# Geo3DSmart/PDANet

Hardware: AMD Instinct MI355X
Metric: scenes/sec (16384-pt ONCE, PDA-SSD forward+backward) (higher is better)
Workload: dtype f32; 1 GPU; once16k_b2_detector_fwd_bwd_adam; scenes_per_gpu=2, global_batch=2, parallelism=dp1, world_size_seen=1, cpu_affinity=GPU-local NUMA node of 0000:d9:00.0: 128 CPUs, full=False, graph_tail=False, graph_head=True

## Files before the change

include/pda_pointnet2.h:

```cpp
#ifndef PDA_POINTNET2_H
#define PDA_POINTNET2_H

#include <stdint.h>

#ifdef __cplusplus
extern "C" {
#endif

#define PDA_OK 0
#define PDA_ERR_INVALID_ARGUMENT 1
#define PDA_ERR_LAUNCH 2
#define PDA_ERR_UNSUPPORTED 3

typedef void *pda_stream_t;

#define PDA_POINTNET2_ABI_VERSION 20
int pda_abi_version(void);
const char *pda_last_error(void);
int pda_fp_contract_mode(void);
int pda_opt_n_threads(int work_size);
int pda_fps_coop_timeouts(unsigned long long *total, int reset);
int pda_debug_fps_spin_limit(int polls);
long long pda_debug_fps_exchange_nonzero(void);

// ... 25 lines not shown
int pda_group_points(const float *points, const int32_t *idx, float *out, int b, int c, int n,
                     int npoints, int nsample, pda_stream_t stream);
int pda_group_points_grad(const float *grad_out, const int32_t *idx, float *grad_points, int b,
                          int c, int n, int npoints, int nsample, pda_stream_t stream);

int pda_group_rows(const float *rows, const int32_t *idx, float *out, int b, int n, int c,
                   int64_t num_idx, pda_stream_t stream);
int pda_group_rows_grad(const float *grad_out, const int32_t *idx, float *grad_rows, int b, int n,
                        int c, int64_t num_idx, pda_stream_t stream);

int pda_three_nn(const float *unknown, const float *known, float *dist2, int32_t *idx, int b,
                 int n, int m, pda_stream_t stream);
int pda_three_interpolate(const float *points, const int32_t *idx, const float *weight,
                          float *out, int b, int c, int m, int n, pda_stream_t stream);
int pda_three_interpolate_grad(const float *grad_out, const int32_t *idx, const float *weight,
                               float *grad_points, int b, int c, int n, int m,
                               pda_stream_t stream);

int pda_chamfer_forward(const float *xyz1, const float *xyz2, float *dist1, float *dist2,
                        int32_t *idx1, int32_t *idx2, int b, int n, int m, pda_stream_t stream);
int pda_chamfer_backward(const float *xyz1, const float *xyz2, float *gradxyz1, float *gradxyz2,
                         const float *graddist1, const float *graddist2, const int32_t *idx1,
                         const int32_t *idx2, int b, int n, int m, pda_stream_t stream);

int pda_group_attention_fwd(const float *qkv, float *out, float *lse, int64_t num_groups, int seq,
                            int heads, int head_dim, pda_stream_t stream);
int pda_group_attention_bwd(const float *qkv, const float *grad_out, const float *lse,
                            float *grad_qkv, int64_t num_groups, int seq, int heads, int head_dim,
                            pda_stream_t stream);
int pda_group_attention_fwd_bf16(const uint16_t *qkv, uint16_t *out, float *lse, int64_t num_groups, int seq,
                                 int heads, int head_dim, pda_stream_t stream);
int pda_group_attention_bwd_bf16(const uint16_t *qkv, const uint16_t *grad_out, const float *lse,
                                 uint16_t *grad_qkv, int64_t num_groups, int seq, int heads, int head_dim,
                                 pda_stream_t stream);

int pda_sa_mlp_maxpool(const float *xyz, const float *new_xyz, const float *features,
                       const int32_t *idx, float *out, int b, int n, int m, int c, int nsample,
                       const int32_t *dims, const float *const *wf, const float *const *scale,
                       const float *const *shift, pda_stream_t stream);
int pda_linear_cols_packed_size(int n_out, int k);
int pda_linear_cols_pack(const float *w, float *wf, int n_out, int k, int transposed_source, int gather_order,
                         pda_stream_t stream);
int pda_linear_cols(const float *x, const float *wf, float *y, int64_t tokens, int k, int n_out, pda_stream_t stream);
int pda_sa_gather_linear(const float *xyz, const float *new_xyz, const float *feats_pm, const int32_t *idx,
                         const float *wf, float *y, int b, int n, int m, int c, int nsample, int n_out,
                         pda_stream_t stream);
int64_t pda_linear_split_packed_bytes(int n_out, int k);
int pda_linear_split_pack(const float *w, void *wf, int n_out, int k, int transposed_source, pda_stream_t stream);
int pda_linear_split_pack_both(const float *w, void *wf, void *wft, int n_out, int k, pda_stream_t stream);
int pda_linear_split(const float *x, const void *wf, const float *bias, float *y, int64_t tokens, int k, int n_out,
                     int relu, pda_stream_t stream);
int pda_gemm_split(const float *x, const void *wf, const float *bias, float *y, int64_t tokens, int k, int n_out,
                   int relu, int accumulate, pda_stream_t stream);
int pda_sa_mlp_packed_size(int rows, int cols, int first_layer);
int pda_sa_mlp_pack_weights(const float *w, float *wf, int rows, int cols, int first_layer,
                            pda_stream_t stream);

#ifdef __cplusplus
}
#endif
#endif
```

include/pda_train.h:

```cpp
#ifndef PDA_TRAIN_H
#define PDA_TRAIN_H
#include "pda_pointnet2.h"

#ifdef __cplusplus
extern "C" {
#endif

int pda_grad_norm(const float *g, int64_t n, float *norm_out, float *scratch1024, pda_stream_t stream);
int pda_adam_onecycle_step(float *p, const float *g, float *m, float *v, int64_t n, float lr,
                           float beta1, float beta2, float eps, float wd, int step,
                           const float *total_norm, float max_norm, pda_stream_t stream);

int64_t pda_bn_relu_scratch_bytes(int c);
int pda_bn_relu_fwd(const float *x, const float *gamma, const float *beta, float *running_mean,
                    float *running_var, float *y, float *mean_invstd, void *scratch, int64_t rows, int c,
                    float eps, float momentum, pda_stream_t stream);
int pda_bn_relu_bwd(const float *x, const float *grad_y, const float *gamma, const float *beta,
                    const float *mean_invstd, float *grad_x, float *grad_gamma, float *grad_beta,
                    void *scratch, int64_t rows, int c, pda_stream_t stream);
int pda_bn_relu_fwd_mixed(const void *x, int x_is_bf16, const float *gamma, const float *beta, float *running_mean,
                          float *running_var, void *y, int y_is_bf16, float *mean_invstd, void *scratch,
                          int64_t rows, int c, float eps, float momentum, pda_stream_t stream);
int pda_bn_relu_bwd_mixed(const void *x, int x_is_bf16, const void *grad_y, int grad_y_is_bf16, const float *gamma,
                          const float *beta, const float *mean_invstd, void *grad_x, float *grad_gamma,
                          float *grad_beta, void *scratch, int64_t rows, int c, pda_stream_t stream);
int pda_bn_relu_max_pool_fwd(const void *x, int x_is_bf16, const float *gamma, const float *beta, float *running_mean,
                             float *running_var, float *out, uint8_t *arg, float *mean_invstd, void *scratch,
                             int64_t groups, int ns, int c, float eps, float momentum, pda_stream_t stream);
int pda_bn_relu_max_pool_bwd(const void *x, int x_is_bf16, const float *grad_out, const uint8_t *arg,
                             const float *gamma, const float *beta, const float *mean_invstd, void *grad_x,
                             float *grad_gamma, float *grad_beta, void *scratch, int64_t groups, int ns, int c,
                             pda_stream_t stream);

int64_t pda_layer_norm_scratch_bytes(int d);
int pda_layer_norm_fwd(const float *x, const float *residual, const float *gamma, const float *beta,
                       float *sum_out, float *y, float *mean_rstd, int64_t rows, int d, float eps,
                       pda_stream_t stream);
int pda_layer_norm_bwd(const float *x, const float *grad_y, const float *grad_y2, const float *gamma,
                       const float *mean_rstd, float *grad_x, float *grad_gamma, float *grad_beta,
                       void *scratch, int64_t rows, int d, pda_stream_t stream);
int pda_layer_norm_fwd_mixed(const void *x, int x_is_bf16, const float *residual, const float *gamma,
                             const float *beta, float *sum_out, float *y, uint16_t *y_bf16, float *mean_rstd,
                             int64_t rows, int d, float eps, pda_stream_t stream);
int pda_layer_norm_bwd_mixed(const float *x, const float *grad_y, const void *grad_y2, int grad_y2_is_bf16,
                             const float *gamma, const float *mean_rstd, float *grad_x, uint16_t *grad_x_bf16,
                             float *grad_gamma, float *grad_beta, void *scratch, int64_t rows, int d,
                             pda_stream_t stream);

int64_t pda_linear_wgrad_scratch_bytes(int64_t tokens, int in_features, int out_features);
int pda_linear_wgrad_form(int64_t tokens, int in_features, int out_features);
int pda_linear_wgrad(const float *x, const float *grad_out, float *grad_weight, float *grad_bias,
                     void *scratch, int64_t tokens, int in_features, int out_features, pda_stream_t stream);
int pda_linear_wgrad_bn(const float *x, const float *grad_out, float *grad_weight, float *grad_bias, void *scratch,
                        int64_t tokens, int in_features, int out_features, const float *x_mean_invstd,
                        const float *x_gamma, const float *x_beta, pda_stream_t stream);

int64_t pda_gemm_split_bn_tiles(int64_t tokens);
int pda_gemm_split_bn(const float *x, const void *wf, float *y, int64_t tokens, int k, int n_out,
                      const float *in_mean_invstd, const float *in_gamma, const float *in_beta, int stats_mode,
                      double *partial, pda_stream_t stream);
int pda_gemm_split_maxpool(const float *x, const void *wf, const float *bias, float *out, int64_t tokens, int k, int n_out,
                           int ns, int relu, pda_stream_t stream);
int pda_gemm_split_gather(const float *point_rows, const float *xyz, const float *new_xyz, const int32_t *idx,
                          const float *w1, int ldw1, const float *bias1, const void *wf, const float *bias2, float *y,
                          int b, int n, int m, int ns, int k, int n_out, int relu, pda_stream_t stream);
int pda_bn_stats_fwd(const float *x, float *running_mean, float *running_var, float *mean_invstd, void *scratch,
                     int64_t rows, int c, float eps, float momentum, pda_stream_t stream);
int pda_bn_finalize_fwd(const double *partial, int nblocks, int c, int64_t count, float eps, float momentum,
                        float *mean_invstd, float *running_mean, float *running_var, pda_stream_t stream);
int pda_bn_relu_max_pool_apply(const float *x, const float *gamma, const float *beta, const float *mean_invstd,
                               float *out, uint8_t *arg, int64_t groups, int ns, int c, pda_stream_t stream);

int64_t pda_colsum_scratch_bytes(int cols);
int pda_colsum_bf16(const uint16_t *g, float *out, void *scratch, int64_t rows, int cols, pda_stream_t stream);

int pda_assemble_tokens(const float *rppe, const float *dscale, const float *feats, const int32_t *idx,
                        const float *glob, float *out, int b, int n, int m, int nsample, int c,
                        pda_stream_t stream);
int pda_assemble_tokens_grad(const float *grad_out, const float *dscale, const float *feats, const int32_t *idx,
                             float *grad_rppe, float *grad_dscale, float *grad_feats, float *grad_glob,
                             int b, int n, int m, int nsample, int c, pda_stream_t stream);

int pda_add_max_pool(const float *a, const float *b, float *out, uint8_t *arg, int64_t groups, int seq, int d,
                     pda_stream_t stream);
int pda_max_pool_scatter(const float *grad_out, const uint8_t *arg, float *grad_x, int64_t groups, int seq,
                         int d, pda_stream_t stream);
int pda_add_max_pool_bf16(const float *a, const uint16_t *b, float *out, uint8_t *arg, int64_t groups, int seq,
                          int d, pda_stream_t stream);
int pda_max_pool_scatter_bf16(const float *grad_out, const uint8_t *arg, float *grad_x, uint16_t *grad_x_bf16,
                              int64_t groups, int seq, int d, pda_stream_t stream);

int pda_bn_relu_fwd_weighted(const float *x, const float *gamma, const float *beta, float *running_mean,
                             float *running_var, float *y, float *mean_invstd, void *scratch, int64_t rows, int c,
                             float eps, float momentum, const float *row_weight, int64_t count, pda_stream_t stream);
int pda_bn_relu_bwd_weighted(const float *x, const float *grad_y, const float *gamma, const float *beta,
                             const float *mean_invstd, float *grad_x, float *grad_gamma, float *grad_beta,
                             void *scratch, int64_t rows, int c, const float *row_weight, int64_t count,
                             pda_stream_t stream);

int pda_ragged_plan(const int32_t *idx, int32_t *cnt, int32_t *off, int32_t *rowmap, float *row_weight, int64_t groups,
                    int nsample, pda_stream_t stream);
int pda_assemble_tokens_ragged(const float *rppe, const float *dscale, const float *feats, const int32_t *idx,
                               const float *glob, const int32_t *rowmap, const int32_t *off, float *out,
                               int64_t max_tokens, int b, int n, int m, int nsample, int c, int rppe_compact,
                               pda_stream_t stream);
int pda_assemble_tokens_ragged_grad(const float *grad_out, const float *dscale, const float *feats,
                                    const int32_t *idx, const int32_t *cnt, const int32_t *off, const int32_t *rowmap,
                                    float *grad_rppe, float *grad_dscale, float *grad_feats, float *grad_glob,
// ... 305 lines not shown
```

pdanet_amd/_lib.py:

```python
import ctypes
import os

_HERE = os.path.dirname(os.path.abspath(__file__))
LIB_PATH = os.environ.get("PDA_LIB_PATH") or os.path.join(_HERE, "libpda_pointnet2.so")
ABI_VERSION = 20


class DensityNetScale(ctypes.Structure):
    _fields_ = [("x", ctypes.c_void_p), ("grad_y", ctypes.c_void_p), ("params", ctypes.c_void_p), ("y", ctypes.c_void_p),
                ("stats", ctypes.c_void_p), ("scratch", ctypes.c_void_p), ("running", ctypes.c_void_p * 6),
                ("grad_params", ctypes.c_void_p), ("n", ctypes.c_int64), ("rowmap", ctypes.c_void_p),
                ("row_weight", ctypes.c_void_p), ("n_unique", ctypes.c_void_p), ("nsample", ctypes.c_int),
                ("eps", ctypes.c_float), ("momentum", ctypes.c_float)]


class OnceFrames(ctypes.Structure):
    _fields_ = [("gt_boxes", ctypes.c_void_p), ("gt_name", ctypes.c_void_p), ("gt_offsets", ctypes.c_void_p),
                ("pred_boxes", ctypes.c_void_p), ("pred_score", ctypes.c_void_p), ("pred_name", ctypes.c_void_p),
                ("pred_start", ctypes.c_void_p), ("pred_count", ctypes.c_void_p), ("iou_start", ctypes.c_void_p),
                ("n_gt_total", ctypes.c_int64), ("pred_cap", ctypes.c_int64), ("iou_cap", ctypes.c_int64),
                ("n_frames", ctypes.c_int), ("max_gt", ctypes.c_int), ("max_pred", ctypes.c_int)]


class KittiFrames(ctypes.Structure):
    _fields_ = [(n, ctypes.c_void_p) for n in ("gt_bbox", "gt_loc", "gt_dims", "gt_ry", "gt_alpha", "gt_trunc", "gt_occ",
                                               "gt_name", "gt_offsets", "dt_bbox", "dt_box", "dt_alpha", "dt_score",
                                               "dt_name", "dt_start", "dt_count", "ov_start", "frame_mode")] + \
               [("n_gt_total", ctypes.c_int64), ("det_cap", ctypes.c_int64), ("ov_cap", ctypes.c_int64),
                ("n_frames", ctypes.c_int), ("max_gt", ctypes.c_int), ("max_det", ctypes.c_int)]


PARAM_EPOCH = [0]
WEIGHT_EPOCH = [0]

_vp = ctypes.c_void_p
_i = ctypes.c_int
_f = ctypes.c_float

SIGNATURES = {
    "pda_furthest_point_sampling": [_vp, _vp, _vp, _i, _i, _i, _vp],
    "pda_furthest_point_sampling_with_dist": [_vp, _vp, _vp, _i, _i, _i, _vp],
    "pda_gather_points": [_vp, _vp, _vp, _i, _i, _i, _i, _vp],
    "pda_gather_points_grad": [_vp, _vp, _vp, _i, _i, _i, _i, _vp],
    "pda_ball_query": [_vp, _vp, _vp, _i, _i, _i, _f, _i, _vp],
    "pda_ball_query_dilated": [_vp, _vp, _vp, _i, _i, _i, _f, _f, _i, _vp],
    "pda_ellipsoid_query": [_vp, _vp, _vp, _i, _i, _i, _f, _f, _f, _i, _vp],
    "pda_ball_query_cells_scratch_bytes": [_i, _i],
    "pda_ball_query_cells": [_vp, _vp, ctypes.POINTER(_vp), _i, _i, _i, _i, ctypes.POINTER(_f), ctypes.POINTER(ctypes.c_int32),
                             _vp, ctypes.c_int64, _vp],
    "pda_ball_query_multi": [_vp, _vp, ctypes.POINTER(_vp), _i, _i, _i, _i,
                             ctypes.POINTER(_f), ctypes.POINTER(ctypes.c_int32), _vp],
    "pda_group_points": [_vp, _vp, _vp, _i, _i, _i, _i, _i, _vp],
    "pda_group_points_grad": [_vp, _vp, _vp, _i, _i, _i, _i, _i, _vp],
    "pda_group_rows": [_vp, _vp, _vp, _i, _i, _i, ctypes.c_int64, _vp],
    "pda_group_rows_grad": [_vp, _vp, _vp, _i, _i, _i, ctypes.c_int64, _vp],
    "pda_three_nn": [_vp, _vp, _vp, _vp, _i, _i, _i, _vp],
    "pda_three_interpolate": [_vp, _vp, _vp, _vp, _i, _i, _i, _i, _vp],
    "pda_three_interpolate_grad": [_vp, _vp, _vp, _vp, _i, _i, _i, _i, _vp],
    "pda_chamfer_forward": [_vp, _vp, _vp, _vp, _vp, _vp, _i, _i, _i, _vp],
    "pda_chamfer_backward": [_vp, _vp, _vp, _vp, _vp, _vp, _vp, _vp, _i, _i, _i, _vp],
    "pda_group_attention_fwd": [_vp, _vp, _vp, ctypes.c_int64, _i, _i, _i, _vp],
    "pda_group_attention_bwd": [_vp, _vp, _vp, _vp, ctypes.c_int64, _i, _i, _i, _vp],
    "pda_group_attention_fwd_bf16": [_vp, _vp, _vp, ctypes.c_int64, _i, _i, _i, _vp],
    "pda_group_attention_bwd_bf16": [_vp, _vp, _vp, _vp, ctypes.c_int64, _i, _i, _i, _vp],
    "pda_sa_mlp_maxpool": [_vp, _vp, _vp, _vp, _vp, _i, _i, _i, _i, _i, ctypes.POINTER(ctypes.c_int32),
                           ctypes.POINTER(_vp), ctypes.POINTER(_vp), ctypes.POINTER(_vp), _vp],
    "pda_linear_cols_packed_size": [_i, _i],
    "pda_linear_cols_pack": [_vp, _vp, _i, _i, _i, _i, _vp],
    "pda_linear_cols": [_vp, _vp, _vp, ctypes.c_int64, _i, _i, _vp],
    "pda_sa_gather_linear": [_vp, _vp, _vp, _vp, _vp, _vp, _i, _i, _i, _i, _i, _i, _vp],
    "pda_linear_split_packed_bytes": [_i, _i],
    "pda_linear_split_pack": [_vp, _vp, _i, _i, _i, _vp],
    "pda_linear_split_pack_both": [_vp, _vp, _vp, _i, _i, _vp],
    "pda_linear_split": [_vp, _vp, _vp, _vp, ctypes.c_int64, _i, _i, _i, _vp],
    "pda_gemm_split": [_vp, _vp, _vp, _vp, ctypes.c_int64, _i, _i, _i, _i, _vp],
    "pda_sa_mlp_packed_size": [_i, _i, _i],
    "pda_sa_mlp_pack_weights": [_vp, _vp, _i, _i, _i, _vp],
    "pda_grad_norm": [_vp, ctypes.c_int64, _vp, _vp, _vp],
    "pda_bn_relu_scratch_bytes": [_i],
    "pda_bn_relu_fwd": [_vp, _vp, _vp, _vp, _vp, _vp, _vp, _vp, ctypes.c_int64, _i, _f, _f, _vp],
    "pda_bn_relu_bwd": [_vp, _vp, _vp, _vp, _vp, _vp, _vp, _vp, _vp, ctypes.c_int64, _i, _vp],    "pda_bn_relu_fwd_mixed": [_vp, _i, _vp, _vp, _vp, _vp, _vp, _i, _vp, _vp, ctypes.c_int64, _i, _f, _f, _vp],
    "pda_bn_relu_bwd_mixed": [_vp, _i, _vp, _i, _vp, _vp, _vp, _vp, _vp, _vp, _vp, ctypes.c_int64, _i, _vp],
    "pda_bn_relu_max_pool_fwd": [_vp, _i, _vp, _vp, _vp, _vp, _vp, _vp, _vp, _vp, ctypes.c_int64, _i, _i, _f, _f, _vp],
    "pda_bn_relu_max_pool_bwd": [_vp, _i, _vp, _vp, _vp, _vp, _vp, _vp, _vp, _vp, _vp, ctypes.c_int64, _i, _i, _vp],

    "pda_layer_norm_scratch_bytes": [_i],
    "pda_layer_norm_fwd": [_vp, _vp, _vp, _vp, _vp, _vp, _vp, ctypes.c_int64, _i, _f, _vp],
    "pda_layer_norm_bwd": [_vp, _vp, _vp, _vp, _vp, _vp, _vp, _vp, _vp, ctypes.c_int64, _i, _vp],
    "pda_layer_norm_fwd_mixed": [_vp, _i, _vp, _vp, _vp, _vp, _vp, _vp, _vp, ctypes.c_int64, _i, _f, _vp],
    "pda_layer_norm_bwd_mixed": [_vp, _vp, _vp, _i, _vp, _vp, _vp, _vp, _vp, _vp, _vp, ctypes.c_int64, _i, _vp],
    "pda_linear_wgrad_scratch_bytes": [ctypes.c_int64, _i, _i],
    "pda_linear_wgrad_form": [ctypes.c_int64, _i, _i],
    "pda_linear_wgrad": [_vp, _vp, _vp, _vp, _vp, ctypes.c_int64, _i, _i, _vp],
    "pda_linear_wgrad_bn": [_vp, _vp, _vp, _vp, _vp, ctypes.c_int64, _i, _i, _vp, _vp, _vp, _vp],
    "pda_gemm_split_bn_tiles": [ctypes.c_int64],
    "pda_gemm_split_bn": [_vp, _vp, _vp, ctypes.c_int64, _i, _i, _vp, _vp, _vp, _i, _vp, _vp],
    "pda_gemm_split_maxpool": [_vp, _vp, _vp, _vp, ctypes.c_int64, _i, _i, _i, _i, _vp],
    "pda_gemm_split_gather": [_vp, _vp, _vp, _vp, _vp, _i, _vp, _vp, _vp, _vp, _i, _i, _i, _i, _i, _i, _i, _vp],
    "pda_bn_stats_fwd": [_vp, _vp, _vp, _vp, _vp, ctypes.c_int64, _i, _f, _f, _vp],
    "pda_bn_finalize_fwd": [_vp, _i, _i, ctypes.c_int64, _f, _f, _vp, _vp, _vp, _vp],
    "pda_bn_relu_max_pool_apply": [_vp, _vp, _vp, _vp, _vp, _vp, ctypes.c_int64, _i, _i, _vp],
    "pda_colsum_scratch_bytes": [_i],
    "pda_colsum_bf16": [_vp, _vp, _vp, ctypes.c_int64, _i, _vp],
    "pda_assemble_tokens": [_vp, _vp, _vp, _vp, _vp, _vp, _i, _i, _i, _i, _i, _vp],
    "pda_assemble_tokens_grad": [_vp, _vp, _vp, _vp, _vp, _vp, _vp, _vp, _i, _i, _i, _i, _i, _vp],
    "pda_add_max_pool": [_vp, _vp, _vp, _vp, ctypes.c_int64, _i, _i, _vp],
    "pda_max_pool_scatter": [_vp, _vp, _vp, ctypes.c_int64, _i, _i, _vp],
    "pda_add_max_pool_bf16": [_vp, _vp, _vp, _vp, ctypes.c_int64, _i, _i, _vp],
    "pda_max_pool_scatter_bf16": [_vp, _vp, _vp, _vp, ctypes.c_int64, _i, _i, _vp],
    "pda_ragged_plan": [_vp, _vp, _vp, _vp, _vp, ctypes.c_int64, _i, _vp],
    "pda_assemble_tokens_ragged": [_vp, _vp, _vp, _vp, _vp, _vp, _vp, _vp, ctypes.c_int64, _i, _i, _i, _i, _i, _i, _vp],
    "pda_assemble_tokens_ragged_grad": [_vp, _vp, _vp, _vp, _vp, _vp, _vp, _vp, _vp, _vp, _vp, ctypes.c_int64, _i, _i, _i, _i, _i, _i, _vp],
    "pda_bn_relu_fwd_weighted": [_vp, _vp, _vp, _vp, _vp, _vp, _vp, _vp, ctypes.c_int64, _i, _f, _f, _vp, ctypes.c_int64, _vp],
    "pda_bn_relu_bwd_weighted": [_vp, _vp, _vp, _vp, _vp, _vp, _vp, _vp, _vp, ctypes.c_int64, _i, _vp, ctypes.c_int64, _vp],
    "pda_add_max_pool_ragged": [_vp, _vp, _vp, _vp, _vp, _vp, ctypes.c_int64, _i, _vp],
    "pda_max_pool_scatter_ragged": [_vp, _vp, _vp, _vp, _vp, ctypes.c_int64, ctypes.c_int64, _i, _i, _vp],
    "pda_group_attention_ragged_fwd": [_vp, _vp, _vp, _vp, _vp, ctypes.c_int64, ctypes.c_int64, _i, _i, _i, _vp],
    "pda_group_attention_ragged_bwd": [_vp, _vp, _vp, _vp, _vp, _vp, ctypes.c_int64, ctypes.c_int64, _i, _i, _i, _vp],
    "pda_densitynet_param_count": [],
    "pda_densitynet_eval_param_count": [],
    "pda_densitynet_scratch_bytes": [],
    "pda_densitynet_fwd": [_vp, _vp, _vp, _vp, _vp, _vp, _vp, _vp, _vp, _vp, _vp, ctypes.c_int64, _f, _f, _vp],
    "pda_densitynet_bwd": [_vp, _vp, _vp, _vp, _vp, _vp, ctypes.c_int64, _f, _vp],
    "pda_densitynet_eval": [_vp, _vp, _vp, ctypes.c_int64, _vp],
    "pda_densitynet_fwd_multi": [_vp, _i, _vp],
    "pda_densitynet_bwd_multi": [_vp, _i, _vp],
    "pda_densitynet_fwd_unique": [_vp, _vp, _vp, _vp, _vp, _vp, _vp, _vp, _vp, _vp, _vp, ctypes.c_int64, _vp, _vp, _vp, _i, _f, _f, _vp],
    "pda_densitynet_bwd_unique": [_vp, _vp, _vp, _vp, _vp, _vp, ctypes.c_int64, _vp, _vp, _vp, _i, _f, _vp],
    "pda_pda_geometry": [_vp, _vp, _vp, _vp, _vp, _i, _i, _i, _i, _f, _vp],
    "pda_points_in_boxes": [_vp, _vp, _vp, _i, _i, _i, _vp],
    "pda_roiaware_pool3d_fwd": [_vp, _vp, _vp, _vp, _vp, _vp, _i, _i, _i, _i, _i, _i, _i, _i, _vp],
    "pda_roiaware_pool3d_bwd": [_vp, _vp, _vp, _vp, _i, _i, _i, _i, _i, _i, _i, _i, _vp],
    "pda_roipoint_pool3d_fwd": [_vp, _vp, _vp, _vp, _vp, _i, _i, _i, _i, _i, _vp],
    "pda_points_in_boxes_mask": [_vp, _vp, _vp, _i, _i, _vp],
    "pda_assign_point_targets": [_vp, _vp, _vp, _vp, _vp, _vp, _i, _i, _i, _i, _i, _vp],
    "pda_sa_gaussian_mask": [_vp, _i, _i, _vp, _vp, _vp, ctypes.c_int64, _vp],
    "pda_head_assign_targets": [_vp, _i, _i, _vp, ctypes.POINTER(ctypes.c_float), _vp, _vp, _vp, _vp, _vp, _i, _i, _i, _i, _i, _i, _vp],
    "pda_head_cls_loss": [_vp, _i, _i, _i, _vp, _vp, ctypes.c_int64, _f, _vp, _vp, _vp],
    "pda_head_centerness": [_vp, _vp, _vp, _vp, ctypes.c_int64, _vp],
    "pda_head_box_loss": [_vp, _vp, _vp, _vp, _f, _i, _f, _f, ctypes.c_int64, _vp, _vp, _vp],
    "pda_head_vote_loss": [_i, _vp, _vp, _vp, _vp, _i, _i, _i, _f, ctypes.c_int64, _vp, _vp, _vp],
    "pda_head_corner_loss": [_vp, _vp, _vp, _i, _vp, _vp, _vp, _i, _f, ctypes.c_int64, _vp, _vp, _vp, _vp],
    "pda_boxes_overlap_bev": [_vp, _vp, _vp, _i, _i, _vp],
    "pda_boxes_iou_bev": [_vp, _vp, _vp, _i, _i, _vp],
    "pda_nms_mask_words": [_i],
    "pda_nms_bev": [_vp, _vp, _vp, _vp, _vp, _i, _i, _f, _i, _vp],
    "pda_sa_small_train_workspace_bytes": [],
# ... 161 lines not shown
```

pdanet_amd/csrc/gemm_split.hip:

```cpp
#include "pda_common.h"
#include "split_bf16.h"

#include <stdlib.h>

namespace pda {

constexpr int GS_MAX_N = 2048;
constexpr int GS_KSTEP = 12 * 64;

__device__ __forceinline__ void split_pack_one(const float* __restrict__ w, uint32_t* __restrict__ wf, int64_t o, int rows, int cols,
                                               int KS, int trans) {
    const int pr = (int)(o & 3), lane = (int)((o >> 2) & 63);
    int64_t rest = o >> 8;
    const int rb = (int)(rest & 3); rest >>= 2;
    const int s = (int)(rest % KS), c = (int)(rest / KS);
    const int row = c * 128 + rb * 32 + (lane & 31);
    const int k = 16 * s + 8 * (lane >> 5) + 2 * pr;
    float v[2];
    for (int e = 0; e < 2; ++e)
        v[e] = (row < rows && k + e < cols) ? (trans ? w[(size_t)(k + e) * rows + row] : w[(size_t)row * cols + k + e]) : 0.f;
    uint32_t h, m, l;
    split2(v[0], v[1], h, m, l);
    const size_t base = ((((size_t)c * KS + s) * 4 + rb) * 3) * 256 + (size_t)lane * 4 + pr;
    wf[base] = h; wf[base + 256] = m; wf[base + 512] = l;
}

__global__ void split_pack_kernel(const float* __restrict__ w, uint32_t* __restrict__ wf, int rows, int cols, int KS,
                                  int chunks, int trans) {
    const int64_t total = (int64_t)chunks * KS * 4 * 64 * 4;
    for (int64_t o = blockIdx.x * (int64_t)blockDim.x + threadIdx.x; o < total; o += (int64_t)gridDim.x * blockDim.x)
        split_pack_one(w, wf, o, rows, cols, KS, trans);
}

__global__ void split_pack_both_kernel(const float* __restrict__ w, uint32_t* __restrict__ wf, uint32_t* __restrict__ wft, int n_out,
                                       int k, int KS, int chunks, int KSt, int chunks_t) {
    const int64_t total = (int64_t)chunks * KS * 4 * 64 * 4, total_t = (int64_t)chunks_t * KSt * 4 * 64 * 4;
    for (int64_t o = blockIdx.x * (int64_t)blockDim.x + threadIdx.x; o < total + total_t; o += (int64_t)gridDim.x * blockDim.x) {
        if (o < total) split_pack_one(w, wf, o, n_out, k, KS, 0);
        else split_pack_one(w, wft, o - total, k, n_out, KSt, 1);
    }
}

struct LinSplitParams {
    const float* x;
    const uint4* wf;
    const float* bias;
    float* y;
    int64_t tokens;
    int k, n_out, chunks, relu;
    int cpb;
    unsigned long long* dbg;
};
#ifdef GS_PROFILE
#define GS_MARK(i) do { if (tid == 0) p.dbg[(size_t)blockIdx.x * 16 + (i)] = __builtin_readcyclecounter(); } while (0)
#else
#define GS_MARK(i) do {} while (0)
#endif

template <int KS>
__global__ __launch_bounds__(256) __attribute__((amdgpu_waves_per_eu(1, 1)))
void lin_split_kernel(const LinSplitParams p) {
    constexpr int G = KS % 4 == 0 ? 4 : 2;
    constexpr int TILE = G * GS_KSTEP;
    constexpr int NG = KS / G;
    constexpr int NLD = TILE / 256;
    __shared__ uint4 ring[3 * TILE];
    __shared__ float bias_s[GS_MAX_N];
    const int tid = threadIdx.x, lane = tid & 63, w = __builtin_amdgcn_readfirstlane(tid >> 6);
    const int h = lane >> 5, j = lane & 31;
    const int64_t tok0 = ((int64_t)blockIdx.x * 4 + w) * 32;
    const int64_t tk = tok0 + j < p.tokens ? tok0 + j : p.tokens - 1;
    const uint4* src = p.wf + tid;
    const int ntiles = p.chunks * NG;
    const int c0 = (int)blockIdx.y * p.cpb, c1 = min(p.chunks, c0 + p.cpb);
    const uint32_t ring_base = (uint32_t)(uintptr_t)(__attribute__((address_space(3))) void*)ring + w * 1024;
    auto issue = [&](int t, int slot) {
        const uint4* g = src + (size_t)(t < ntiles ? t : ntiles - 1) * TILE;
        const uint32_t l = ring_base + slot * (TILE * 16);
#pragma unroll
        for (int i = 0; i < NLD; ++i) glds16(g + 256 * i, l + 4096 * i);
    };
    static_assert(NLD <= G * 4, "one DMA instruction per MFMA group at most");
    GS_MARK(0);
    float x[KS * 8];
    {
        const float* row = p.x + tk * p.k + 8 * h;
#pragma unroll
        for (int s = 0; s < KS; ++s) {
            const float4 a = *reinterpret_cast<const float4*>(row + 16 * s), b = *reinterpret_cast<const float4*>(row + 16 * s + 4);
            x[8 * s] = a.x; x[8 * s + 1] = a.y; x[8 * s + 2] = a.z; x[8 * s + 3] = a.w;
            x[8 * s + 4] = b.x; x[8 * s + 5] = b.y; x[8 * s + 6] = b.z; x[8 * s + 7] = b.w;
        }
    }
    for (int i = tid; i < p.n_out; i += 256) bias_s[i] = p.bias ? p.bias[i] : 0.f;
    asm volatile("s_waitcnt vmcnt(0)" ::: "memory");
    GS_MARK(1);
    issue(c0 * NG, 0);
    issue(c0 * NG + 1, 1);
    asm volatile("s_waitcnt vmcnt(%0)" ::"n"(NLD) : "memory");
    __builtin_amdgcn_s_barrier();
    GS_MARK(2);
    const uint32_t lane_off = (uint32_t)(4 * h * p.n_out + j);
    const int64_t left = p.tokens - tok0 - 4 * h;
    const bool whole = tok0 + 32 <= p.tokens;
    auto store_one = [&](const gs_f32x16 (&res)[4], int chunk, int n) {
        const int r = n >> 4, i = n & 15, t = (i & 3) + 8 * (i >> 2);
        float v = res[r][i] + bias_s[chunk * 128 + r * 32 + j];
        if (p.relu) v = fmaxf(v, 0.f);
        float* row = p.y + (tok0 + t) * p.n_out + chunk * 128 + r * 32;
        if (whole) row[lane_off] = v;
        else if (t < left) row[lane_off] = v;
    };
    int ti = c0 * NG, slot = 0;
    gs_f32x16 done[4];
    for (int c = c0; c < c1; ++c) {
        gs_f32x16 acc[4];
#pragma unroll
        for (int r = 0; r < 4; ++r)
#pragma unroll
            for (int i = 0; i < 16; ++i) acc[r][i] = 0.f;
#pragma unroll
        for (int g = 0; g < NG; ++g, ++ti, slot = slot == 2 ? 0 : slot + 1) {
            if (c == 1 && g == 0) GS_MARK(4);
            const uint4* dsrc = src + (size_t)(ti + 2 < ntiles ? ti + 2 : ntiles - 1) * TILE;
            const uint32_t ddst = ring_base + (slot == 0 ? 2 : slot - 1) * (TILE * 16);
            if (c == 1 && g == 0) GS_MARK(5);
            const uint4* buf = ring + slot * TILE + lane;
            uint4 fa[2][3];
#pragma unroll
            for (int pl = 0; pl < 3; ++pl) fa[0][pl] = buf[pl * 64];
#pragma unroll
            for (int sl = 0; sl < G; ++sl) {
                const int s = g * G + sl;
                if constexpr (KS > 16) {
#pragma unroll
                    for (int q = 0; q < 8; ++q) asm volatile("" : "+v"(x[8 * s + q]));
                }
                uint32_t bh[4], bm[4], bl[4];
#pragma unroll
                for (int q = 0; q < 4; ++q) split2(x[8 * s + 2 * q], x[8 * s + 2 * q + 1], bh[q], bm[q], bl[q]);
                const gs_bf16x8 Xh = __builtin_bit_cast(gs_bf16x8, make_uint4(bh[0], bh[1], bh[2], bh[3]));
                const gs_bf16x8 Xm = __builtin_bit_cast(gs_bf16x8, make_uint4(bm[0], bm[1], bm[2], bm[3]));
                const gs_bf16x8 Xl = __builtin_bit_cast(gs_bf16x8, make_uint4(bl[0], bl[1], bl[2], bl[3]));
#pragma unroll
                for (int r = 0; r < 4; ++r) {
                    const int q = sl * 4 + r;
                    if (q + 1 < G * 4) {
#pragma unroll
                        for (int pl = 0; pl < 3; ++pl) fa[(q + 1) & 1][pl] = buf[((q + 1) * 3 + pl) * 64];
                    }
                    __builtin_amdgcn_sched_barrier(0);
                    const gs_bf16x8 Wh = __builtin_bit_cast(gs_bf16x8, fa[q & 1][0]);
                    const gs_bf16x8 Wm = __builtin_bit_cast(gs_bf16x8, fa[q & 1][1]);
                    const gs_bf16x8 Wl = __builtin_bit_cast(gs_bf16x8, fa[q & 1][2]);
                    acc[r] = __builtin_amdgcn_mfma_f32_32x32x16_bf16(Xl, Wh, acc[r], 0, 0, 0);
                    acc[r] = __builtin_amdgcn_mfma_f32_32x32x16_bf16(Xh, Wl, acc[r], 0, 0, 0);
                    acc[r] = __builtin_amdgcn_mfma_f32_32x32x16_bf16(Xm, Wm, acc[r], 0, 0, 0);
                    acc[r] = __builtin_amdgcn_mfma_f32_32x32x16_bf16(Xm, Wh, acc[r], 0, 0, 0);
                    acc[r] = __builtin_amdgcn_mfma_f32_32x32x16_bf16(Xh, Wm, acc[r], 0, 0, 0);
                    acc[r] = __builtin_amdgcn_mfma_f32_32x32x16_bf16(Xh, Wh, acc[r], 0, 0, 0);
                    if (q < NLD) glds16(dsrc + 256 * q, ddst + 4096 * q);
                    if (c > c0) {
                        constexpr int GROUPS = KS * 4;
                        const int gq = g * G * 4 + q;
#pragma unroll
                        for (int n = gq * 64 / GROUPS; n < (gq + 1) * 64 / GROUPS; ++n) store_one(done, c - 1, n);
                    }
                    __builtin_amdgcn_sched_barrier(0);
                }
            }
            if (c == 1 && g == 0) GS_MARK(6);
            asm volatile("s_waitcnt vmcnt(%0)" ::"n"(NLD) : "memory");
            if (c == 1 && g == 0) GS_MARK(7);
            __builtin_amdgcn_s_barrier();
            if (c == 1 && g == 0) GS_MARK(8);
            if (c == 0 && g == NG - 1) GS_MARK(3);
        }
#pragma unroll
        for (int r = 0; r < 4; ++r) done[r] = acc[r];
    }
    GS_MARK(9);
#pragma unroll
    for (int n = 0; n < 64; ++n) store_one(done, c1 - 1, n);
    GS_MARK(10);
}

struct GemmSplitParams {
    const float* x;
    const uint4* wf;
    const float* bias;
    float* y;
    int64_t tokens;
    int k, n_out, chunks, ksteps, relu, accum;
    const float* in_mi;
    const float* in_g;
    const float* in_b;
    double* partial;
    int pool_ns;
    const int32_t* g_idx;
    const float* g_xyz;
    const float* g_ctr;
    const float* g_w;
    const float* g_bias;
    int gn, g_ns, g_m, g_ldw;
};

constexpr int GT_XCHUNKS = 128 * 4;
constexpr int GT_SLOT = GT_XCHUNKS + GS_KSTEP;
constexpr int GW_TILE_U4 = (8 + 8) * 192;

__global__ __launch_bounds__(256, 2)
void gemm_split_kernel(const GemmSplitParams p) {
    __shared__ uint4 ring[3 * GT_SLOT];
    const int tid = threadIdx.x, lane = tid & 63, w = __builtin_amdgcn_readfirstlane(tid >> 6);
    const int h = lane >> 5, r = lane & 31;
    const int wt = w & 1, wo = w >> 1;
    const int nc = (int)(blockIdx.x % (unsigned)p.chunks);
    const int64_t tok0 = (int64_t)(blockIdx.x / (unsigned)p.chunks) * 128;
    const uint32_t ring_base = (uint32_t)(uintptr_t)(__attribute__((address_space(3))) void*)ring;
    const float* xsrc[2];
#pragma unroll
    for (int e = 0; e < 2; ++e) {
        const int pch = 64 * (2 * w + e) + lane, row = pch >> 2, cl = pch & 3, c = cl ^ ((row >> 2) & 3);
        const int64_t tok = tok0 + row < p.tokens ? tok0 + row : p.tokens - 1;
        xsrc[e] = p.x + tok * p.k + 4 * c;
    }
    const uint4* wsrc = p.wf + (size_t)nc * p.ksteps * GS_KSTEP + 64 * 3 * w + lane;
    auto issue = [&](int s, int slot) {
        const int ss = s < p.ksteps ? s : p.ksteps - 1;
        const uint32_t base = ring_base + slot * (GT_SLOT * 16);
#pragma unroll
        for (int e = 0; e < 2; ++e) glds16(reinterpret_cast<const uint4*>(xsrc[e] + 16 * ss), base + (2 * w + e) * 1024);
#pragma unroll
        for (int e = 0; e < 3; ++e) glds16(wsrc + (size_t)ss * GS_KSTEP + 64 * e, base + GT_XCHUNKS * 16 + (3 * w + e) * 1024);
    };
    gs_f32x16 acc[2][2];
#pragma unroll
    for (int a = 0; a < 2; ++a)
#pragma unroll
        for (int b = 0; b < 2; ++b)
#pragma unroll
            for (int i = 0; i < 16; ++i) acc[a][b][i] = 0.f;
    int xoff[2][2];
#pragma unroll
    for (int tt = 0; tt < 2; ++tt) {
        const int row = wt * 64 + tt * 32 + r;
// ... 12 lines not shown
        const uint4* buf = ring + slot * GT_SLOT;
        uint4 wfr[2][3];
#pragma unroll
        for (int ot = 0; ot < 2; ++ot)
#pragma unroll
            for (int pl = 0; pl < 3; ++pl) wfr[ot][pl] = buf[woff + (ot * 3 + pl) * 64];
#pragma unroll
        for (int tt = 0; tt < 2; ++tt) {
            const uint4 a = buf[xoff[tt][0]], b = buf[xoff[tt][1]];
            uint32_t bh[4], bm[4], bl[4];
#ifdef GS_NOSPLIT
            bh[0] = a.x; bh[1] = a.y; bh[2] = a.z; bh[3] = a.w; bm[0] = b.x; bm[1] = b.y; bm[2] = b.z; bm[3] = b.w;
            bl[0] = a.x ^ b.x; bl[1] = a.y ^ b.y; bl[2] = a.z ^ b.z; bl[3] = a.w ^ b.w;
#else
            split2(__uint_as_float(a.x), __uint_as_float(a.y), bh[0], bm[0], bl[0]);
            split2(__uint_as_float(a.z), __uint_as_float(a.w), bh[1], bm[1], bl[1]);
            split2(__uint_as_float(b.x), __uint_as_float(b.y), bh[2], bm[2], bl[2]);
            split2(__uint_as_float(b.z), __uint_as_float(b.w), bh[3], bm[3], bl[3]);
#endif
            const gs_bf16x8 Xh = __builtin_bit_cast(gs_bf16x8, make_uint4(bh[0], bh[1], bh[2], bh[3]));
            const gs_bf16x8 Xm = __builtin_bit_cast(gs_bf16x8, make_uint4(bm[0], bm[1], bm[2], bm[3]));
            const gs_bf16x8 Xl = __builtin_bit_cast(gs_bf16x8, make_uint4(bl[0], bl[1], bl[2], bl[3]));
#pragma unroll
            for (int ot = 0; ot < 2; ++ot) {
                const gs_bf16x8 Wh = __builtin_bit_cast(gs_bf16x8, wfr[ot][0]);
                const gs_bf16x8 Wm = __builtin_bit_cast(gs_bf16x8, wfr[ot][1]);
                const gs_bf16x8 Wl = __builtin_bit_cast(gs_bf16x8, wfr[ot][2]);
                gs_f32x16 c = acc[tt][ot];
                c = __builtin_amdgcn_mfma_f32_32x32x16_bf16(Xl, Wh, c, 0, 0, 0);
                c = __builtin_amdgcn_mfma_f32_32x32x16_bf16(Xh, Wl, c, 0, 0, 0);
                c = __builtin_amdgcn_mfma_f32_32x32x16_bf16(Xm, Wm, c, 0, 0, 0);
                c = __builtin_amdgcn_mfma_f32_32x32x16_bf16(Xm, Wh, c, 0, 0, 0);
                c = __builtin_amdgcn_mfma_f32_32x32x16_bf16(Xh, Wm, c, 0, 0, 0);
                c = __builtin_amdgcn_mfma_f32_32x32x16_bf16(Xh, Wh, c, 0, 0, 0);
                acc[tt][ot] = c;
            }
        }
    }
    asm volatile("s_waitcnt vmcnt(0)" ::: "memory");
#pragma unroll
    for (int ot = 0; ot < 2; ++ot) {
        const int col = nc * 128 + (wo * 2 + ot) * 32 + r;
        if (col >= p.n_out) continue;
        const float bias = p.bias ? p.bias[col] : 0.f;
#pragma unroll
        for (int tt = 0; tt < 2; ++tt) {
            const int64_t trow = tok0 + wt * 64 + tt * 32 + 4 * h;
#pragma unroll
            for (int i = 0; i < 16; ++i) {
                const int64_t tok = trow + (i & 3) + 8 * (i >> 2);
                if (tok < p.tokens) {
                    float* dst = p.y + tok * p.n_out + col;
                    float v = acc[tt][ot][i] + bias;
                    if (p.accum) v += *dst;
                    if (p.relu) v = fmaxf(v, 0.f);
#ifdef GS_NOSTORE
                    if (v == 12345.678f)
#endif
                    *dst = v;
                }
            }
        }
    }
}

typedef uint32_t gp_u32x4 __attribute__((ext_vector_type(4)));

template <int PRO, int EPI>
__global__ __launch_bounds__(512, 1)
void gemm_split_wide_kernel(const GemmSplitParams p) {
    constexpr int TW = 4;
    constexpr int XF = 2 * TW;
    constexpr int NP = 24 / (2 * TW);
    constexpr int TILE_U4 = GW_TILE_U4;
    extern __shared__ uint4 gp_planes[];
    const int tid = threadIdx.x, lane = tid & 63, w = __builtin_amdgcn_readfirstlane(tid >> 6);
    const int h = lane >> 5, r = lane & 31;
    const int wt = w % TW, wo = w / TW;
    const int wide_chunks = (p.chunks + 1) >> 1;
    const int ncb = (int)(blockIdx.x % (unsigned)wide_chunks);
    const int64_t tok0 = (int64_t)(blockIdx.x / (unsigned)wide_chunks) * (64 * TW);
    const int64_t ptok = tok0 + 32 * w + r < p.tokens ? tok0 + 32 * w + r : p.tokens - 1;
    const float* xsrc = p.x + ptok * p.k + 8 * h;
    float gdx = 0.f, gdy = 0.f, gdz = 0.f;
    if constexpr (PRO == 2) {
        const int64_t grp = ptok / p.g_ns;
        const int64_t prow = (grp / p.g_m) * p.gn + p.g_idx[ptok];
        xsrc = p.x + prow * p.k + 8 * h;
        const float* pt = p.g_xyz + prow * 3;
        const float* ct = p.g_ctr + grp * 3;
        gdx = pt[0] - ct[0]; gdy = pt[1] - ct[1]; gdz = pt[2] - ct[2];
    }
    const uint4* wsrc[NP];
#pragma unroll
    for (int e = 0; e < NP; ++e) {
        const int piece = NP * w + e, half = piece / 12, j = piece - 12 * half;
        int chunk = 2 * ncb + half;
        if (chunk >= p.chunks) chunk = p.chunks - 1;
        wsrc[e] = p.wf + (size_t)chunk * p.ksteps * GS_KSTEP + 64 * j + lane;
    }
    auto wld = [&](int e, int ss) { return *reinterpret_cast<const gp_u32x4*>(wsrc[e] + (size_t)ss * GS_KSTEP); };
    auto wst = [&](uint4* dst, const gp_u32x4& v) { *reinterpret_cast<gp_u32x4*>(dst) = v; };
    auto load = [&](int st, float4 (&x)[2], gp_u32x4 (&wv)[NP]) {
        const int ss = st < p.ksteps ? st : p.ksteps - 1;
        x[0] = *reinterpret_cast<const float4*>(xsrc + 16 * ss);
        x[1] = *reinterpret_cast<const float4*>(xsrc + 16 * ss + 4);
#pragma unroll
// ... 135 lines not shown
    if constexpr (EPI == 2) {
        const int ns = p.pool_ns;
#pragma unroll
        for (int ot = 0; ot < 4; ++ot) {
            const int col = (2 * ncb + wo) * 128 + ot * 32 + r;
            const float bias = (p.bias && col < p.n_out) ? p.bias[col] : 0.f;
            float g16[4];
#pragma unroll
            for (int tt = 0; tt < 2; ++tt)
#pragma unroll
                for (int half = 0; half < 2; ++half) {
                    float m = -__builtin_inff();
#pragma unroll
                    for (int i = 8 * half; i < 8 * half + 8; ++i) {
                        float v = acc[tt][ot][i] + bias;
                        if (p.relu) v = fmaxf(v, 0.f);
                        m = fmaxf(m, v);
                    }
                    g16[2 * tt + half] = fmaxf(m, __shfl_xor(m, 32));
                }
            if (h == 0 && col < p.n_out) {
                const int64_t t0 = tok0 + wt * 64;
                if (ns == 16) {
#pragma unroll
                    for (int q = 0; q < 4; ++q)
                        if (t0 + 16 * q < p.tokens) p.y[((t0 + 16 * q) >> 4) * p.n_out + col] = g16[q];
                } else if (ns == 32) {
#pragma unroll
                    for (int q = 0; q < 2; ++q)
                        if (t0 + 32 * q < p.tokens) p.y[((t0 + 32 * q) >> 5) * p.n_out + col] = fmaxf(g16[2 * q], g16[2 * q + 1]);
                } else if (t0 < p.tokens) {
                    p.y[(t0 >> 6) * p.n_out + col] = fmaxf(fmaxf(g16[0], g16[1]), fmaxf(g16[2], g16[3]));
                }
            }
        }
        return;
    }
    double cs1[4], cs2[4];
#pragma unroll
    for (int ot = 0; ot < 4; ++ot) {
        cs1[ot] = 0; cs2[ot] = 0;
        const int col = (2 * ncb + wo) * 128 + ot * 32 + r;
        if (col >= p.n_out) continue;
        const float bias = p.bias ? p.bias[col] : 0.f;
#pragma unroll
        for (int tt = 0; tt < 2; ++tt) {
            const int64_t trow = tok0 + wt * 64 + tt * 32 + 4 * h;
#pragma unroll
            for (int i = 0; i < 16; ++i) {
                const int64_t tok = trow + (i & 3) + 8 * (i >> 2);
                if (tok < p.tokens) {
                    float* dst = p.y + tok * p.n_out + col;
                    float v = acc[tt][ot][i] + bias;
                    if (p.accum) v += *dst;
                    if (p.relu) v = fmaxf(v, 0.f);
#ifdef GS_NOSTORE
                    if (v == 12345.678f)
#endif
                    *dst = v;
                    if constexpr (EPI == 1) { cs1[ot] += v; cs2[ot] += (double)v * v; }
                }
            }
        }
    }
    if constexpr (EPI == 1) {
        double* red = reinterpret_cast<double*>(gp_planes);
        __syncthreads();
#pragma unroll
        for (int ot = 0; ot < 4; ++ot) {
            const double a = cs1[ot] + __shfl_xor(cs1[ot], 32), b = cs2[ot] + __shfl_xor(cs2[ot], 32);
            if (h == 0) {
                const int cl = wo * 128 + ot * 32 + r;
                red[(wt * 256 + cl) * 2] = a; red[(wt * 256 + cl) * 2 + 1] = b;
            }
        }
        __syncthreads();
        if (tid < 256) {
            const int col = 2 * ncb * 128 + tid;
            if (col < p.n_out) {
                double a = 0, b = 0;
#pragma unroll
                for (int q = 0; q < TW; ++q) { a += red[(q * 256 + tid) * 2]; b += red[(q * 256 + tid) * 2 + 1]; }
                double* pp = p.partial + (size_t)(blockIdx.x / (unsigned)wide_chunks) * 2 * p.n_out;
                pp[col] = a; pp[p.n_out + col] = b;
            }
        }
    }
}

}

PDA_API int64_t pda_linear_split_packed_bytes(int n_out, int k) {
    if (n_out <= 0 || k <= 0) return 0;
    return (int64_t)pda::divup(n_out, 128) * pda::divup(k, 32) * 2 * 12 * 64 * 16;
}

PDA_API int pda_linear_split_pack(const float* w, void* wf, int n_out, int k, int transposed_source, pda_stream_t stream) {
    PDA_REQUIRE(w && wf && n_out > 0 && k > 0, "pda_linear_split_pack: bad argument");
    const int chunks = pda::divup(n_out, 128), KS = pda::divup(k, 32) * 2;
    const int64_t total = (int64_t)chunks * KS * 4 * 64 * 4;
    const int blocks = (int)(pda::divup64(total, 256) < 2048 ? pda::divup64(total, 256) : 2048);
    hipLaunchKernelGGL(pda::split_pack_kernel, dim3(blocks), dim3(256), 0, (hipStream_t)stream, w, (uint32_t*)wf, n_out, k, KS,
                       chunks, transposed_source);
    return pda::check_launch("pda_linear_split_pack");
}

PDA_API int pda_linear_split_pack_both(const float* w, void* wf, void* wft, int n_out, int k, pda_stream_t stream) {
    PDA_REQUIRE(w && wf && wft && n_out > 0 && k > 0, "pda_linear_split_pack_both: bad argument");
    const int chunks = pda::divup(n_out, 128), KS = pda::divup(k, 32) * 2;
    const int chunks_t = pda::divup(k, 128), KSt = pda::divup(n_out, 32) * 2;
    const int64_t total = ((int64_t)chunks * KS + (int64_t)chunks_t * KSt) * 4 * 64 * 4;
    const int blocks = (int)(pda::divup64(total, 256) < 2048 ? pda::divup64(total, 256) : 2048);
    hipLaunchKernelGGL(pda::split_pack_both_kernel, dim3(blocks), dim3(256), 0, (hipStream_t)stream, w, (uint32_t*)wf, (uint32_t*)wft,
                       n_out, k, KS, chunks, KSt, chunks_t);
    return pda::check_launch("pda_linear_split_pack_both");
}

PDA_API int pda_linear_split(const float* x, const void* wf, const float* bias, float* y, int64_t tokens, int k, int n_out,
                             int relu, pda_stream_t stream) {
    PDA_REQUIRE(tokens >= 0 && k > 0 && n_out > 0, "pda_linear_split: bad size");
    if (tokens == 0) return PDA_OK;
    PDA_REQUIRE(x && wf && y && (((uintptr_t)x | (uintptr_t)wf | (uintptr_t)y | (uintptr_t)bias) & 15) == 0,
                "pda_linear_split: null or misaligned pointer");
    if (k % 32 != 0 || k > 512 || n_out % 128 != 0 || n_out > pda::GS_MAX_N) {
        pda::set_error("pda_linear_split: no kernel built for K=%d, N=%d (K a multiple of 32 <= 512, N a multiple of 128 <= 2048)", k, n_out);
        return PDA_ERR_UNSUPPORTED;
    }
    pda::LinSplitParams p{};
    p.x = x; p.wf = (const uint4*)wf; p.bias = bias; p.y = y; p.tokens = tokens; p.k = k; p.n_out = n_out; p.chunks = n_out / 128;
    p.relu = relu;
#ifdef GS_PROFILE
    p.dbg = (unsigned long long*)bias; p.bias = nullptr;
#endif
    const int64_t tiles = pda::divup64(tokens, 128);
    const int want = tiles >= 192 ? 1 : (int)pda::divup64(256, tiles);
    p.cpb = pda::divup(p.chunks, want < p.chunks ? want : p.chunks);
    const dim3 grid((unsigned)tiles, (unsigned)pda::divup(p.chunks, p.cpb)), block(256);
    const hipStream_t s = (hipStream_t)stream;
    switch (k / 16) {
#define PDA_GS_CASE(KS) case KS: hipLaunchKernelGGL((pda::lin_split_kernel<KS>), grid, block, 0, s, p); break
        PDA_GS_CASE(2); PDA_GS_CASE(4); PDA_GS_CASE(6); PDA_GS_CASE(8); PDA_GS_CASE(12); PDA_GS_CASE(16); PDA_GS_CASE(24); PDA_GS_CASE(32);
#undef PDA_GS_CASE
        default:
            pda::set_error("pda_linear_split: no kernel built for K=%d", k);
            return PDA_ERR_UNSUPPORTED;
    }
    return pda::check_launch("pda_linear_split");
}

PDA_API int pda_gemm_split(const float* x, const void* wf, const float* bias, float* y, int64_t tokens, int k, int n_out,
                           int relu, int accumulate, pda_stream_t stream) {
    PDA_REQUIRE(tokens >= 0 && k > 0 && n_out > 0, "pda_gemm_split: bad size");
    if (tokens == 0) return PDA_OK;
    PDA_REQUIRE(x && wf && y && (((uintptr_t)x | (uintptr_t)wf) & 15) == 0, "pda_gemm_split: null or misaligned pointer");
    if (k % 16 != 0) {
        pda::set_error("pda_gemm_split: K=%d must be a multiple of 16", k);
        return PDA_ERR_UNSUPPORTED;
    }
    pda::GemmSplitParams p{};
    p.x = x; p.wf = (const uint4*)wf; p.bias = bias; p.y = y; p.tokens = tokens; p.k = k; p.n_out = n_out;
    p.chunks = pda::divup(n_out, 128); p.ksteps = pda::divup(k, 32) * 2; p.relu = relu; p.accum = accumulate;
    const int64_t blocks = pda::divup64(tokens, 128) * p.chunks;
    PDA_REQUIRE(blocks < (1ll << 31), "pda_gemm_split: too many tiles");
    const int packed_steps = p.ksteps;
    p.ksteps = k / 16;
    if (packed_steps != p.ksteps) {
        pda::set_error("pda_gemm_split: K=%d must be a multiple of 32 (packed planes come in pairs of K steps)", k);
        return PDA_ERR_UNSUPPORTED;
    }
    static const int force = getenv("PDA_GEMM_SPLIT_TILE") ? atoi(getenv("PDA_GEMM_SPLIT_TILE")) : 0;
    const int64_t wide_blocks = pda::divup64(tokens, 256) * ((p.chunks + 1) / 2);
    if (force == 256 || (force != 128 && wide_blocks >= 200 && (p.chunks % 2 == 0 || p.chunks >= 5))) {
        static pda::PerDevice<bool> lds_ok;
        const bool ok = lds_ok.get([] { return hipFuncSetAttribute((const void*)pda::gemm_split_wide_kernel<0, 0>, hipFuncAttributeMaxDynamicSharedMemorySize,
                                                                   2 * pda::GW_TILE_U4 * 16) == hipSuccess; });
        if (ok) {
            hipLaunchKernelGGL((pda::gemm_split_wide_kernel<0, 0>), dim3((unsigned)wide_blocks), dim3(512), 2 * pda::GW_TILE_U4 * 16,
                               (hipStream_t)stream, p);
            return pda::check_launch("pda_gemm_split");
        }
    }
    hipLaunchKernelGGL(pda::gemm_split_kernel, dim3((unsigned)blocks), dim3(256), 0, (hipStream_t)stream, p);
    return pda::check_launch("pda_gemm_split");
}

PDA_API int64_t pda_gemm_split_bn_tiles(int64_t tokens) { return tokens > 0 ? pda::divup64(tokens, 256) : 0; }

PDA_API int pda_gemm_split_bn(const float* x, const void* wf, float* y, int64_t tokens, int k, int n_out, const float* in_mean_invstd,
                              const float* in_gamma, const float* in_beta, int stats_mode, double* partial, pda_stream_t stream) {
    PDA_REQUIRE(tokens >= 1 && k > 0 && n_out > 0, "pda_gemm_split_bn: bad size");
    PDA_REQUIRE(x && wf && y && (((uintptr_t)x | (uintptr_t)wf) & 15) == 0, "pda_gemm_split_bn: null or misaligned pointer");
    const bool pro = in_mean_invstd != nullptr;
    PDA_REQUIRE(pro == (in_gamma != nullptr) && pro == (in_beta != nullptr), "pda_gemm_split_bn: the input BatchNorm needs mean_invstd, gamma and beta");
    PDA_REQUIRE(stats_mode >= 0 && stats_mode <= 1 && (stats_mode == 0 || partial), "pda_gemm_split_bn: stats_mode=%d (0 or 1; 1 needs `partial`)", stats_mode);
    if (k % 32 != 0 || k > 1024) {
        pda::set_error("pda_gemm_split_bn: no kernel built for K=%d (a multiple of 32, <= 1024)", k);
        return PDA_ERR_UNSUPPORTED;
    }
    pda::GemmSplitParams p{};
    p.x = x; p.wf = (const uint4*)wf; p.y = y; p.tokens = tokens; p.k = k; p.n_out = n_out;
    p.chunks = pda::divup(n_out, 128); p.ksteps = k / 16;
    p.in_mi = in_mean_invstd; p.in_g = in_gamma; p.in_b = in_beta; p.partial = partial;
    const int64_t wide_blocks = pda::divup64(tokens, 256) * ((p.chunks + 1) / 2);
    PDA_REQUIRE(wide_blocks < (1ll << 31), "pda_gemm_split_bn: too many tiles");
    const int lds = 2 * pda::GW_TILE_U4 * 16 + (pro ? k * 16 : 0);
    const void* fn;
    if (pro && stats_mode == 1) fn = (const void*)pda::gemm_split_wide_kernel<1, 1>;
    else if (pro && stats_mode == 0) fn = (const void*)pda::gemm_split_wide_kernel<1, 0>;
    else if (stats_mode == 1) fn = (const void*)pda::gemm_split_wide_kernel<0, 1>;
    else fn = (const void*)pda::gemm_split_wide_kernel<0, 0>;
    static pda::PerDevice<bool> lds_ok[4];
    const bool ok = lds_ok[(pro ? 2 : 0) + stats_mode].get([fn] {
        return hipFuncSetAttribute(fn, hipFuncAttributeMaxDynamicSharedMemorySize, 2 * pda::GW_TILE_U4 * 16 + 1024 * 16) == hipSuccess; });
    PDA_REQUIRE(ok, "pda_gemm_split_bn: dynamic LDS refused");
    void* args[] = {(void*)&p};
    PDA_REQUIRE(hipLaunchKernel(fn, dim3((unsigned)wide_blocks), dim3(512), args, lds, (hipStream_t)stream) == hipSuccess,
                "pda_gemm_split_bn: launch failed");
    return pda::check_launch("pda_gemm_split_bn");
}

PDA_API int pda_gemm_split_maxpool(const float* x, const void* wf, const float* bias, float* out, int64_t tokens, int k, int n_out, int ns,
                                   int relu, pda_stream_t stream) {
    PDA_REQUIRE(tokens >= 0 && k > 0 && n_out > 0, "pda_gemm_split_maxpool: bad size");
// ... 46 lines not shown
```

pdanet_amd/csrc/wgrad.hip:

```cpp
#include "pda_common.h"
#include "split_bf16.h"

#include <stdlib.h>

namespace pda {

typedef float f32x16 __attribute__((ext_vector_type(16)));

constexpr int WG_KC = 32;
constexpr int WG_TILE = 128;

__device__ __forceinline__ void lds_dma16(const float* gsrc, float* lds_dst_wave_uniform) {
    uint32_t keep;
    const uint32_t dst = __builtin_amdgcn_readfirstlane((uint32_t)(uintptr_t)lds_dst_wave_uniform);
    asm volatile("s_mov_b32 %0, m0\n\ts_mov_b32 m0, %2\n\ts_nop 0\n\tglobal_load_lds_dwordx4 %1, off\n\ts_mov_b32 m0, %0"
                 : "=&s"(keep) : "v"(gsrc), "s"(dst) : "memory");
}

__global__ __launch_bounds__(256) void wgrad_kernel(const float* __restrict__ X, const float* __restrict__ G,
                                                    float* __restrict__ part_w, float* __restrict__ part_b, int64_t T, int M,
                                                    int N, int tiles_m, int tiles_n, int S, int64_t KS, int nblocks) {
    __shared__ __attribute__((aligned(16))) float ldsG[2][WG_KC][WG_TILE];
    __shared__ __attribute__((aligned(16))) float ldsX[2][WG_KC][WG_TILE];
    const int per_xcd = (nblocks + 7) / 8;
    const int logical = (int)(blockIdx.x & 7) * per_xcd + (int)(blockIdx.x >> 3);
    if (logical >= nblocks) return;
    const int tiles = tiles_m * tiles_n;
    const int tile = logical % tiles, s = logical / tiles;
    const int n0 = (tile / tiles_m) * WG_TILE, m0 = (tile % tiles_m) * WG_TILE;
    const int64_t t_begin = (int64_t)s * KS, t_end = (t_begin + KS < T) ? t_begin + KS : T;

    const int tid = threadIdx.x, lane = lane_id(), w = wave_id();
    const int c = lane & 31, h = lane >> 5;
    const int wn = w >> 1, wm = w & 1;
    const int lrow = tid >> 5, lcol = (tid & 31) * 4;
    const bool g_ok = n0 + lcol < N, x_ok = m0 + lcol < M;

    f32x16 acc[2][2];
#pragma unroll
    for (int i = 0; i < 2; ++i)
#pragma unroll
        for (int j = 0; j < 2; ++j)
#pragma unroll
            for (int r = 0; r < 16; ++r) acc[i][j][r] = 0.f;
    float bsum[2] = {0.f, 0.f};

    float4 rg[4], rx[4];
    const int gcol = g_ok ? n0 + lcol : 0, xcol = x_ok ? m0 + lcol : 0;
    auto load_chunk = [&](int64_t t0) {
#pragma unroll
        for (int p = 0; p < 4; ++p) {
            const int64_t t = t0 + p * 8 + lrow;
            const bool in = t < t_end;
            const int64_t tc = in ? t : t_end - 1;
            const float4 vg = *reinterpret_cast<const float4*>(G + tc * N + gcol);
            const float4 vx = *reinterpret_cast<const float4*>(X + tc * M + xcol);
            rg[p] = (in && g_ok) ? vg : make_float4(0.f, 0.f, 0.f, 0.f);
            rx[p] = (in && x_ok) ? vx : make_float4(0.f, 0.f, 0.f, 0.f);
        }
    };
    auto store_chunk = [&](int buf) {
#pragma unroll
        for (int p = 0; p < 4; ++p) {
            *reinterpret_cast<float4*>(&ldsG[buf][p * 8 + lrow][lcol]) = rg[p];
            *reinterpret_cast<float4*>(&ldsX[buf][p * 8 + lrow][lcol]) = rx[p];
        }
    };

    const bool full_tile = (n0 + WG_TILE <= N) && (m0 + WG_TILE <= M);
    auto dma_chunk = [&](int64_t t0, int b) {
#pragma unroll
        for (int i = 0; i < 4; ++i) {
            const int row = w * 8 + 2 * i;
            const int64_t t = t0 + row + (lane >> 5);
            const int col = (lane & 31) * 4;
            lds_dma16(G + t * N + n0 + col, &ldsG[b][row][0]);
            lds_dma16(X + t * M + m0 + col, &ldsX[b][row][0]);
        }
// ... 22 lines not shown

    int buf = 0;
    int64_t t0 = t_begin;
    if (full_tile) {
        const int64_t n_full = (t_end - t_begin) / WG_KC;
        if (n_full > 0) {
            dma_chunk(t_begin, 0);
            asm volatile("s_waitcnt vmcnt(0)" ::: "memory");
            __syncthreads();
            for (int64_t i = 0; i < n_full; ++i) {
                if (i + 1 < n_full) dma_chunk(t_begin + (i + 1) * WG_KC, buf ^ 1);
                compute(buf);
                asm volatile("s_waitcnt vmcnt(0)" ::: "memory");
                __syncthreads();
                buf ^= 1;
            }
            t0 = t_begin + n_full * WG_KC;
        }
    }
    if (t0 < t_end) {
        load_chunk(t0);
        store_chunk(buf);
        __syncthreads();
        for (; t0 < t_end; t0 += WG_KC) {
            const bool more = t0 + WG_KC < t_end;
            if (more) load_chunk(t0 + WG_KC);
            compute(buf);
            if (more) store_chunk(buf ^ 1);
            __syncthreads();
            buf ^= 1;
        }
    }

    float* pw = part_w + (size_t)s * N * M;
#pragma unroll
    for (int i = 0; i < 2; ++i)
#pragma unroll
        for (int j = 0; j < 2; ++j) {
            const int m = m0 + wm * 64 + j * 32 + c;
#pragma unroll
            for (int r = 0; r < 16; ++r) {
                const int n = n0 + wn * 64 + i * 32 + (r & 3) + 8 * (r >> 2) + 4 * h;
                if (n < N && m < M) pw[(size_t)n * M + m] = acc[i][j][r];
            }
        }
    if (part_b && m0 == 0 && wm == 0) {
#pragma unroll
        for (int i = 0; i < 2; ++i) {
            const float v = bsum[i] + __shfl_xor(bsum[i], 32);
            const int n = n0 + wn * 64 + i * 32 + c;
            if (h == 0 && n < N) part_b[(size_t)s * N + n] = v;
        }
    }
}

#ifndef WSP_ABL
#define WSP_ABL 0
#endif
constexpr int WSP_TILE_U4 = 2 * 8 * 3 * 64;

template <bool XBN>
__global__ __launch_bounds__(512, 1)
void wgrad_split_kernel(const float* __restrict__ X, const float* __restrict__ G, float* __restrict__ part_w,
                        float* __restrict__ part_b, int64_t T, int M, int N, int tiles_m, int tiles_n, int S, int64_t KS,
                        int nblocks, const float* __restrict__ x_mi, const float* __restrict__ x_g, const float* __restrict__ x_b) {
    extern __shared__ uint4 wsp_planes[];
    const int per_xcd = (nblocks + 7) / 8;
    const int logical = (int)(blockIdx.x & 7) * per_xcd + (int)(blockIdx.x >> 3);
    if (logical >= nblocks) return;
    const int tiles = tiles_m * tiles_n;
    const int tile = logical % tiles, s = logical / tiles;
    const int n0 = (tile / tiles_m) * 256, m0 = (tile % tiles_m) * 256;
    const int64_t t_begin = (int64_t)s * KS, t_end = (t_begin + KS < T) ? t_begin + KS : T;
    const int len = (int)(t_end - t_begin), ksteps = (len + 15) >> 4;

    const int tid = threadIdx.x, lane = tid & 63, w = __builtin_amdgcn_readfirstlane(tid >> 6);
    const int c = lane & 31, h = lane >> 5;
    const int wn = w >> 1, wm = w & 1;
    const uint32_t span_g = (uint32_t)((((int64_t)len - 1) * N + 32) * 4), span_x = (uint32_t)((((int64_t)len - 1) * M + 32) * 4);
    const __amdgpu_buffer_rsrc_t rg = __builtin_amdgcn_make_buffer_rsrc((void*)(G + t_begin * N + n0 + 32 * w), 0, span_g, 0x00020000);
    const __amdgpu_buffer_rsrc_t rx = __builtin_amdgcn_make_buffer_rsrc((void*)(X + t_begin * M + m0 + 32 * w), 0, span_x, 0x00020000);
    const int vg = (8 * h * N + c) * 4, vx = (8 * h * M + c) * 4;
    auto load1 = [&](int st, int j, float (&g)[8], float (&x)[8]) {
        g[j] = __builtin_bit_cast(float, __builtin_amdgcn_raw_buffer_load_b32(rg, vg, (16 * st + j) * N * 4, 0));
        x[j] = __builtin_bit_cast(float, __builtin_amdgcn_raw_buffer_load_b32(rx, vx, (16 * st + j) * M * 4, 0));
    };
    auto load = [&](int st, float (&g)[8], float (&x)[8]) {
#pragma unroll
        for (int j = 0; j < 8; ++j) load1(st, j, g, x);
    };
    float xmu = 0.f, xis = 0.f, xga = 0.f, xbe = 0.f;
    if constexpr (XBN) { const int m = m0 + 32 * w + c; xmu = x_mi[m]; xis = x_mi[M + m]; xga = x_g[m]; xbe = x_b[m]; }
    auto xt = [&](float v) { return XBN ? fmaxf((v - xmu) * xis * xga + xbe, 0.f) : v; };
    float bsum = 0.f;
    const bool do_bias = part_b && m0 == 0;
    gs_f32x16 acc[2][4];
#pragma unroll
    for (int a = 0; a < 2; ++a)
#pragma unroll
        for (int b = 0; b < 4; ++b)
#pragma unroll
            for (int i = 0; i < 16; ++i) acc[a][b][i] = 0.f;
    const int aoff = (2 * wn) * 192 + lane, boff = (8 + 4 * wm) * 192 + lane;
    uint4* const my_planes = wsp_planes + w * 192 + lane;

    gs_bf16x8 Bf[2][3];
    constexpr int PA[6] = {2, 0, 1, 1, 0, 0}, PB[6] = {0, 2, 1, 0, 1, 0};
    auto step = [&](int st, const float (&ga)[8], const float (&xa)[8], float (&gb)[8], float (&xb)[8],
                    const gs_bf16x8 (&Ap)[2][3], gs_bf16x8 (&An)[2][3]) {
#if WSP_ABL != 4
        __syncthreads();
#endif
        const uint4* buf = wsp_planes + (st & 1) * WSP_TILE_U4;
        uint4* out = my_planes + ((st + 1) & 1) * WSP_TILE_U4;
#pragma unroll
        for (int i = 0; i < 2; ++i)
#pragma unroll
            for (int pl = 0; pl < 3; ++pl) An[i][pl] = __builtin_bit_cast(gs_bf16x8, buf[aoff + i * 192 + pl * 64]);
        auto read_b = [&](int jt) {
#pragma unroll
            for (int pl = 0; pl < 3; ++pl) Bf[jt & 1][pl] = __builtin_bit_cast(gs_bf16x8, buf[boff + jt * 192 + pl * 64]);
// ... 57 lines not shown
#endif
        }
    };
    auto split_store = [&](const float (&g)[8], const float (&x)[8], int b) {
        uint4* out = my_planes + b * WSP_TILE_U4;
        uint32_t ph[4], pm[4], pl[4];
#pragma unroll
        for (int q = 0; q < 4; ++q) split2(g[2 * q], g[2 * q + 1], ph[q], pm[q], pl[q]);
        out[0] = make_uint4(ph[0], ph[1], ph[2], ph[3]);
        out[64] = make_uint4(pm[0], pm[1], pm[2], pm[3]);
        out[128] = make_uint4(pl[0], pl[1], pl[2], pl[3]);
#pragma unroll
        for (int q = 0; q < 4; ++q) split2(xt(x[2 * q]), xt(x[2 * q + 1]), ph[q], pm[q], pl[q]);
        out[8 * 192] = make_uint4(ph[0], ph[1], ph[2], ph[3]);
        out[8 * 192 + 64] = make_uint4(pm[0], pm[1], pm[2], pm[3]);
        out[8 * 192 + 128] = make_uint4(pl[0], pl[1], pl[2], pl[3]);
        bsum += ((g[0] + g[1]) + (g[2] + g[3])) + ((g[4] + g[5]) + (g[6] + g[7]));
    };
    float g1[8], x1[8], g2[8], x2[8];
    gs_bf16x8 A0[2][3], A1[2][3];
#pragma unroll
    for (int i = 0; i < 2; ++i)
#pragma unroll
        for (int pl = 0; pl < 3; ++pl) {
            A0[i][pl] = __builtin_bit_cast(gs_bf16x8, make_uint4(0u, 0u, 0u, 0u));
            Bf[1][pl] = A0[i][pl];
        }
    load(0, g1, x1);
    split_store(g1, x1, 0);
    load(1, g1, x1);
    for (int st = 0; st < ksteps; st += 2) {
        step(st, g1, x1, g2, x2, A0, A1);
        step(st + 1, g2, x2, g1, x1, A1, A0);
    }
#pragma unroll
    for (int e = 0; e < 12; ++e)
        acc[e & 1][3] = __builtin_amdgcn_mfma_f32_32x32x16_bf16(A0[e & 1][PA[e >> 1]], Bf[1][PB[e >> 1]], acc[e & 1][3], 0, 0, 0);
    float* pw = part_w + (size_t)s * N * M;
#pragma unroll
    for (int i = 0; i < 2; ++i)
#pragma unroll
        for (int jt = 0; jt < 4; ++jt) {
            const int m = m0 + 128 * wm + 32 * jt + c;
#pragma unroll
            for (int r = 0; r < 16; ++r) {
                const int n = n0 + 64 * wn + 32 * i + (r & 3) + 8 * (r >> 2) + 4 * h;
                pw[(size_t)n * M + m] = acc[i][jt][r];
            }
        }
    if (do_bias) {
        const float v = bsum + __shfl_xor(bsum, 32);
        if (h == 0) part_b[(size_t)s * N + n0 + 32 * w + c] = v;
    }
}

__device__ __forceinline__ float sum_slices(const float* __restrict__ part, int S, int64_t stride, int64_t e, bool live, int slice,
                                            float (*red)[64], int el) {
    float a = 0.f;
    if (live) {
        float v[8];
        for (int s0 = slice; s0 < S; s0 += 16 * 8) {
#pragma unroll
            for (int u = 0; u < 8; ++u) {
                const int sidx = s0 + 16 * u;
                v[u] = sidx < S ? part[(size_t)sidx * stride + e] : 0.f;
            }
#pragma unroll
            for (int u = 0; u < 8; ++u) a += v[u];
        }
    }
    red[slice][el] = a;
    __syncthreads();
    float r = 0.f;
    if (slice == 0)
#pragma unroll
        for (int p = 0; p < 16; ++p) r += red[p][el];
    __syncthreads();
    return r;
}

__global__ __launch_bounds__(1024) void wgrad_reduce_kernel(const float* __restrict__ part_w, const float* __restrict__ part_b,
                                                            float* __restrict__ dw, float* __restrict__ db, int S, int64_t nm, int N) {
    __shared__ float red[16][64];
    const int el = threadIdx.x & 63, slice = threadIdx.x >> 6;
    const int64_t e = (int64_t)blockIdx.x * 64 + el;
    const float w = sum_slices(part_w, S, nm, e, e < nm, slice, red, el);
    if (slice == 0 && e < nm) dw[e] = w;
    if (db && (int64_t)blockIdx.x * 64 < N) {
        const float bsum = sum_slices(part_b, S, N, e, e < N, slice, red, el);
        if (slice == 0 && e < N) db[e] = bsum;
    }
}

constexpr int WS_UNROLL = 8;
constexpr int WS_MAX_SLICES = 1024;

template <int NT, int MT>
__global__ __launch_bounds__(256) void wgrad_skinny_kernel(const float* __restrict__ X, const float* __restrict__ G,
                                                           float* __restrict__ part_w, float* __restrict__ part_b, int64_t T, int M,
                                                           int N, int64_t KS) {
    __shared__ float red[NT * MT * 1024 + 64 * NT];
    const int tid = threadIdx.x, lane = lane_id(), w = wave_id();
    const int i = lane & 31, h = lane >> 5;
    const int64_t t_begin = (int64_t)blockIdx.x * KS, t_end = (t_begin + KS < T) ? t_begin + KS : T;
    f32x16 acc[NT][MT];
    float sb[NT];
// ... 67 lines not shown
    KS = divup64(divup64(T, s), 8) * 8;
    S = (int)divup64(T, KS);
}

static void wgrad_plan(int64_t T, int M, int N, int& tiles_m, int& tiles_n, int& S, int64_t& KS) {
    tiles_m = divup(M, WG_TILE); tiles_n = divup(N, WG_TILE);
    const int tiles = tiles_m * tiles_n;
    int64_t s = 512 / tiles;
    if (T / s < 128 && tiles <= 256) s = 256 / tiles;
    const int64_t max_s = T / 64 > 0 ? T / 64 : 1;
    if (s > max_s) s = max_s;
    if (s < 1) s = 1;
    KS = divup64(divup64(T, s), WG_KC) * WG_KC;
    S = (int)divup64(T, KS);
}

static bool wgrad_use_split(int64_t T, int M, int N) {
    static const int mode = [] { const char* e = getenv("PDA_WGRAD_SPLIT"); return e ? atoi(e) : 1; }();
    if (mode == 0 || (M & 255) || (N & 255) || T < 4096) return false;
    return mode == 2 || (double)T * M * N >= 2.0e9;
}
static void wgrad_split_plan(int64_t T, int M, int N, int& tiles_m, int& tiles_n, int& S, int64_t& KS) {
    tiles_m = M / 256; tiles_n = N / 256;
    const int tiles = tiles_m * tiles_n;
    int64_t s = 256 / tiles;
    const int64_t max_s = T / 256 > 0 ? T / 256 : 1;
    if (s > max_s) s = max_s;
    const int64_t min_s = divup64(T * (M > N ? M : N) * 4, (int64_t)1 << 31);
    if (s < min_s) s = min_s;
    if (s < 1) s = 1;
    KS = divup64(divup64(T, s), 16) * 16;
    S = (int)divup64(T, KS);
}

}

PDA_API int64_t pda_linear_wgrad_scratch_bytes(int64_t tokens, int in_features, int out_features) {
    if (tokens <= 0 || in_features <= 0 || out_features <= 0) return 0;
    int tm, tn, S;
    int64_t KS;
    if (pda::wgrad_is_skinny(in_features, out_features)) pda::wgrad_skinny_plan(tokens, S, KS);
    else if (pda::wgrad_use_split(tokens, in_features, out_features)) pda::wgrad_split_plan(tokens, in_features, out_features, tm, tn, S, KS);
    else pda::wgrad_plan(tokens, in_features, out_features, tm, tn, S, KS);
    return (int64_t)S * ((int64_t)in_features * out_features + out_features) * (int64_t)sizeof(float);
}

PDA_API int pda_linear_wgrad_form(int64_t tokens, int in_features, int out_features) {
    if (pda::wgrad_is_skinny(in_features, out_features)) return 1;
    return pda::wgrad_use_split(tokens, in_features, out_features) ? 2 : 0;
}

namespace pda {
static int linear_wgrad(const float* x, const float* grad_out, float* grad_weight, float* grad_bias, void* scratch, int64_t tokens,
                        int in_features, int out_features, pda_stream_t stream, const float* x_mi, const float* x_g, const float* x_b);
}

PDA_API int pda_linear_wgrad(const float* x, const float* grad_out, float* grad_weight, float* grad_bias, void* scratch,
                             int64_t tokens, int in_features, int out_features, pda_stream_t stream) {
    return pda::linear_wgrad(x, grad_out, grad_weight, grad_bias, scratch, tokens, in_features, out_features, stream, nullptr, nullptr, nullptr);
}

PDA_API int pda_linear_wgrad_bn(const float* x, const float* grad_out, float* grad_weight, float* grad_bias, void* scratch,
                                int64_t tokens, int in_features, int out_features, const float* x_mean_invstd, const float* x_gamma,
                                const float* x_beta, pda_stream_t stream) {
    PDA_REQUIRE(x_mean_invstd && x_gamma && x_beta, "pda_linear_wgrad_bn: null pointer");
    if (pda_linear_wgrad_form(tokens, in_features, out_features) != 2) {
        pda::set_error("pda_linear_wgrad_bn: tokens=%lld in=%d out=%d does not run on the split form", (long long)tokens, in_features, out_features);
        return PDA_ERR_UNSUPPORTED;
    }
    return pda::linear_wgrad(x, grad_out, grad_weight, grad_bias, scratch, tokens, in_features, out_features, stream, x_mean_invstd, x_gamma, x_beta);
}

int pda::linear_wgrad(const float* x, const float* grad_out, float* grad_weight, float* grad_bias, void* scratch, int64_t tokens,
                             int in_features, int out_features, pda_stream_t stream, const float* x_mi, const float* x_g, const float* x_b) {
    const int M = in_features, N = out_features;
    PDA_REQUIRE(tokens >= 1 && M >= 4 && N >= 4 && (M & 3) == 0 && (N & 3) == 0,
                "pda_linear_wgrad: tokens=%lld in=%d out=%d (features must be multiples of 4)", (long long)tokens, M, N);
    PDA_REQUIRE(x && grad_out && grad_weight && scratch, "pda_linear_wgrad: null pointer");
    PDA_REQUIRE((((uintptr_t)x | (uintptr_t)grad_out) & 15) == 0, "pda_linear_wgrad: x / grad_out must be 16-byte aligned");
    int tm, tn, S;
    int64_t KS;
    hipStream_t st = (hipStream_t)stream;
    if (pda::wgrad_is_skinny(M, N)) {
        pda::wgrad_skinny_plan(tokens, S, KS);
        float* pw = (float*)scratch;
        float* pb = grad_bias ? pw + (size_t)S * N * M : (float*)nullptr;
        const int nt = N > 32 ? 2 : 1, mt = M > 32 ? 2 : 1;
#define PDA_WS_CASE(A, B) hipLaunchKernelGGL((pda::wgrad_skinny_kernel<A, B>), dim3(S), dim3(256), 0, st, x, grad_out, pw, pb, tokens, M, N, KS)
        if (nt == 1 && mt == 1) PDA_WS_CASE(1, 1);
        else if (nt == 1) PDA_WS_CASE(1, 2);
        else if (mt == 1) PDA_WS_CASE(2, 1);
        else PDA_WS_CASE(2, 2);
#undef PDA_WS_CASE
        const int64_t nm = (int64_t)N * M;
        hipLaunchKernelGGL(pda::wgrad_reduce_kernel, dim3((unsigned)pda::divup64(nm, 64)), dim3(1024), 0, st, pw, pb, grad_weight,
                           grad_bias, S, nm, N);
        return pda::check_launch("pda_linear_wgrad");
    }
    if (pda::wgrad_use_split(tokens, M, N)) {
        pda::wgrad_split_plan(tokens, M, N, tm, tn, S, KS);
        const int nblocks = S * tm * tn;
        float* part_w = (float*)scratch;
        float* part_b = part_w + (size_t)S * N * M;
        static pda::PerDevice<bool> lds_ok;
        const bool ok = lds_ok.get([] {
            return hipFuncSetAttribute((const void*)pda::wgrad_split_kernel<false>, hipFuncAttributeMaxDynamicSharedMemorySize, 2 * pda::WSP_TILE_U4 * 16) == hipSuccess &&
                   hipFuncSetAttribute((const void*)pda::wgrad_split_kernel<true>, hipFuncAttributeMaxDynamicSharedMemorySize, 2 * pda::WSP_TILE_U4 * 16) == hipSuccess; });
        PDA_REQUIRE(ok, "pda_linear_wgrad: %d bytes of dynamic LDS refused", 2 * pda::WSP_TILE_U4 * 16);
        if (x_mi)
            hipLaunchKernelGGL(pda::wgrad_split_kernel<true>, dim3(pda::divup(nblocks, 8) * 8), dim3(512), 2 * pda::WSP_TILE_U4 * 16, st,
                               x, grad_out, part_w, grad_bias ? part_b : (float*)nullptr, tokens, M, N, tm, tn, S, KS, nblocks, x_mi, x_g, x_b);
        else
            hipLaunchKernelGGL(pda::wgrad_split_kernel<false>, dim3(pda::divup(nblocks, 8) * 8), dim3(512), 2 * pda::WSP_TILE_U4 * 16, st,
                               x, grad_out, part_w, grad_bias ? part_b : (float*)nullptr, tokens, M, N, tm, tn, S, KS, nblocks, x_mi, x_g, x_b);
        const int64_t nm = (int64_t)N * M;
        hipLaunchKernelGGL(pda::wgrad_reduce_kernel, dim3((unsigned)pda::divup64(nm, 64)), dim3(1024), 0, st, part_w, part_b,
                           grad_weight, grad_bias, S, nm, N);
        return pda::check_launch("pda_linear_wgrad");
    }
    pda::wgrad_plan(tokens, M, N, tm, tn, S, KS);
    const int nblocks = S * tm * tn;
    float* part_w = (float*)scratch;
    float* part_b = part_w + (size_t)S * N * M;
    hipLaunchKernelGGL(pda::wgrad_kernel, dim3(pda::divup(nblocks, 8) * 8), dim3(256), 0, st, x, grad_out, part_w,
                       grad_bias ? part_b : (float*)nullptr, tokens, M, N, tm, tn, S, KS, nblocks);
    const int64_t nm = (int64_t)N * M;
    hipLaunchKernelGGL(pda::wgrad_reduce_kernel, dim3((unsigned)pda::divup64(nm, 64)), dim3(1024), 0, st, part_w, part_b, grad_weight,
                       grad_bias, S, nm, N);
    return pda::check_launch("pda_linear_wgrad");
}

namespace pda {

constexpr int CS_BLOCKS = 512;

__global__ __launch_bounds__(256) void colsum_bf16_kernel(const bf16_t* __restrict__ g, float* __restrict__ partial, int64_t rows,
                                                          int cols, int nv, int rpb) {
    __shared__ float lds[256 * 8];
    const int tid = threadIdx.x;
    float acc[8] = {0.f, 0.f, 0.f, 0.f, 0.f, 0.f, 0.f, 0.f};
    const int v = tid % nv, r0 = tid / nv;
    if (tid < nv * rpb) {
        for (int64_t r = (int64_t)blockIdx.x * rpb + r0; r < rows; r += (int64_t)gridDim.x * rpb) {
            const uint4 u = *reinterpret_cast<const uint4*>(g + r * cols + 8 * v);
            acc[0] += __uint_as_float(u.x << 16); acc[1] += __uint_as_float(u.x & 0xffff0000u);
            acc[2] += __uint_as_float(u.y << 16); acc[3] += __uint_as_float(u.y & 0xffff0000u);
            acc[4] += __uint_as_float(u.z << 16); acc[5] += __uint_as_float(u.z & 0xffff0000u);
            acc[6] += __uint_as_float(u.w << 16); acc[7] += __uint_as_float(u.w & 0xffff0000u);
        }
    }
#pragma unroll
    for (int k = 0; k < 8; ++k) lds[tid * 8 + k] = acc[k];
    __syncthreads();
    if (tid < nv) {
        float s[8] = {0.f, 0.f, 0.f, 0.f, 0.f, 0.f, 0.f, 0.f};
        for (int r = 0; r < rpb; ++r)
#pragma unroll
            for (int k = 0; k < 8; ++k) s[k] += lds[(r * nv + tid) * 8 + k];
#pragma unroll
        for (int k = 0; k < 8; ++k) partial[(size_t)blockIdx.x * cols + 8 * tid + k] = s[k];
    }
}

__global__ __launch_bounds__(256) void colsum_final_kernel(const float* __restrict__ partial, int nblocks, int cols,
                                                           float* __restrict__ out) {
    __shared__ double red[16][16];
    const int cl = threadIdx.x & 15, part = threadIdx.x >> 4;
    const int c = blockIdx.x * 16 + cl;
    double a = 0.0;
    if (c < cols) {
        float va[8];
        for (int k0 = part; k0 < nblocks; k0 += 16 * 8) {
#pragma unroll
            for (int u = 0; u < 8; ++u) {
                const int k = k0 + 16 * u;
                va[u] = k < nblocks ? partial[(size_t)k * cols + c] : 0.f;
            }
#pragma unroll
// ... 30 lines not shown
```

pdanet_amd/optimization.py:

```python
import math

import numpy as np
import torch
from torch import nn

from . import _lib
from . import param_cache

BN_TYPES = (nn.BatchNorm1d, nn.BatchNorm2d, nn.BatchNorm3d, nn.SyncBatchNorm)


def flatten_model(m):
    children = list(m.children())
    return sum((flatten_model(c) for c in children), []) if children else [m]


def trained_parameter_groups(model):
    names = {id(p): n for n, p in model.named_parameters()}
    groups, seen = ([], []), set()
    for leaf in flatten_model(model):
        g = groups[1] if isinstance(leaf, BN_TYPES) else groups[0]
        for p in leaf.parameters():
            if p.requires_grad and id(p) not in seen:
                seen.add(id(p))
                g.append((names.get(id(p), "?"), p))
    return groups


def annealing_cos(start, end, pct):
    cos_out = np.cos(np.pi * pct) + 1
    return end + (start - end) / 2 * cos_out


class OneCycle:

    def __init__(self, optimizer, total_step, lr_max, moms, div_factor, pct_start):
        self.optimizer, self.total_step = optimizer, total_step
        low_lr = lr_max / div_factor
        lr_phases = ((0, (low_lr, lr_max)), (pct_start, (lr_max, low_lr / 1e4)))
        mom_phases = ((0, tuple(moms)), (pct_start, tuple(moms[::-1])))
        self.lr_phases = self._phases(lr_phases)
        self.mom_phases = self._phases(mom_phases)
        optimizer.lr, optimizer.mom = low_lr, moms[0]

    def _phases(self, phases):
        out = []
        for i, (start, ends) in enumerate(phases):
            stop = int(phases[i + 1][0] * self.total_step) if i < len(phases) - 1 else self.total_step
            out.append((int(start * self.total_step), stop, ends))
        return out

    def values(self, step):
        lr = mom = None
        for start, end, (a, b) in self.lr_phases:
            if step >= start:
                lr = annealing_cos(a, b, (step - start) / (end - start))
        for start, end, (a, b) in self.mom_phases:
            if step >= start:
                mom = annealing_cos(a, b, (step - start) / (end - start))
        return float(lr), float(mom)
# ... 17 lines not shown
        for p in everything:
            if p.dtype != torch.float32 or p.device != dev:
                raise _lib.PdaError("FlatAdamOneCycle: fp32 parameters on one device only")
            self.offsets.append(off)
            off += (p.numel() + 3) // 4 * 4
            if p is trained[-1]:
                self.n_trained = off
        self.flat_p = torch.zeros(self.n_trained, device=dev)
        self.flat_g = torch.zeros(off, device=dev)
        self.exp_avg = torch.zeros(self.n_trained, device=dev)
        self.exp_avg_sq = torch.zeros(self.n_trained, device=dev)
        self._norm = torch.zeros(1, device=dev)
        self._scratch = torch.zeros(1024, device=dev)
        for p, o in zip(everything, self.offsets):
            n = p.numel()
            if o < self.n_trained:
                self.flat_p[o:o + n].copy_(p.data.reshape(-1))
                p.data = self.flat_p[o:o + n].view(p.shape)
            p.grad = self.flat_g[o:o + n].view(p.shape)
        self._all = everything
        self._grad_views = [p.grad for p in everything]
        self._gather = False
        self.params = trained
        self.wd, self.beta2, self.eps, self.grad_norm_clip = wd, beta2, eps, grad_norm_clip
        self.lr, self.mom = lr, mom
        self.step_count = 0
        self._dp_group, self._dp_world, self._dp_avg = None, 1, False

    def data_parallel(self, group=None, sync_parameters=True, model=None):
        import torch.distributed as dist
        if not dist.is_initialized() or dist.get_world_size(group) == 1:
            return self
        self._dp_group, self._dp_world = group, dist.get_world_size(group)
        self._dp_avg = False
        if dist.get_backend(group) == "nccl":
            try:
                probe = torch.ones(4, device=self.flat_g.device)
                dist.all_reduce(probe, op=dist.ReduceOp.AVG, group=group)
                self._dp_avg = bool((probe == 1).all().item())
            except (RuntimeError, ValueError):
                self._dp_avg = False
        if sync_parameters:
            src = dist.get_global_rank(group, 0) if group is not None else 0
            dist.broadcast(self.flat_p, src, group=group)
            if model is not None:
                mine = {id(p) for p in self.params}
                for t in [p.data for p in model.parameters() if id(p) not in mine] + list(model.buffers()):
                    dist.broadcast(t, src, group=group)
            param_cache.parameters_written()
        return self

    def exchange_gradients(self):
        import torch.distributed as dist
        if self._gather:
            self._gather_grads()
        if self._dp_world == 1:
            return
        if self._dp_avg:
            dist.all_reduce(self.flat_g, op=dist.ReduceOp.AVG, group=self._dp_group)
        else:
            dist.all_reduce(self.flat_g, op=dist.ReduceOp.SUM, group=self._dp_group)
            self.flat_g.mul_(1.0 / self._dp_world)

    def zero_grad(self, set_to_none=False):
        if set_to_none:
            for p in self._all:
                p.grad = None
            self._gather = True
        else:
            if self._gather:
                for p, v in zip(self._all, self._grad_views):
                    p.grad = v
                self._gather = False
            self.flat_g.zero_()

    def _gather_grads(self):
        self.flat_g.zero_()
        dsts, srcs = [], []
        for p, v in zip(self._all, self._grad_views):
            g = p.grad
            if g is not None and g.data_ptr() != v.data_ptr():
                dsts.append(v); srcs.append(g.detach())
            p.grad = v
        if srcs:
            torch._foreach_copy_(dsts, srcs)
        self._gather = False

    def step(self):
        if self.flat_p.device.type != "cuda":
            raise _lib.PdaError("FlatAdamOneCycle.step needs the parameters on the GPU (no CPU path)")
        lib = _lib.load()
        if self._gather:
            self._gather_grads()
        if self._dp_world > 1:
            self.exchange_gradients()
        stream = torch.cuda.current_stream(self.flat_p.device).cuda_stream
        with torch.cuda.device(self.flat_p.device):
            norm_ptr = None
            if self.grad_norm_clip is not None:
                _lib.check(lib.pda_grad_norm(self.flat_g.data_ptr(), self.flat_g.numel(), self._norm.data_ptr(),
                                             self._scratch.data_ptr(), stream), "pda_grad_norm")
                norm_ptr = self._norm.data_ptr()
            self.step_count += 1
            param_cache.parameters_written()
            _lib.check(lib.pda_adam_onecycle_step(
                self.flat_p.data_ptr(), self.flat_g.data_ptr(), self.exp_avg.data_ptr(), self.exp_avg_sq.data_ptr(),
                self.n_trained, self.lr, self.mom, self.beta2, self.eps, self.wd, self.step_count, norm_ptr,
                float(self.grad_norm_clip or 0.0), stream), "pda_adam_onecycle_step")

    @property
    def total_norm(self):
        return self._norm

    def state_dict(self):
        state, k = {}, 0
        group_params = []
        for g in self.groups:
            idxs = []
            for _, p in g:
                o, n = self.offsets[k], p.numel()
                state[k] = {"step": torch.tensor(float(self.step_count)),
                            "exp_avg": self.exp_avg[o:o + n].view(p.shape).clone(),
                            "exp_avg_sq": self.exp_avg_sq[o:o + n].view(p.shape).clone()}
                idxs.append(k)
                k += 1
            group_params.append(idxs)
        if self.step_count == 0:
            state = {}
        pg = [{"lr": self.lr, "betas": (self.mom, self.beta2), "eps": self.eps, "weight_decay": 0,
               "amsgrad": False, "maximize": False, "foreach": None, "capturable": False,
               "differentiable": False, "fused": None, "params": idxs} for idxs in group_params]
        return {"state": state, "param_groups": pg}

    def load_state_dict(self, sd):
        pg = sd["param_groups"]
        n = sum(len(g["params"]) for g in pg)
        if n != len(self.params):
            raise ValueError("optimizer state has %d parameters, model trains %d" % (n, len(self.params)))
        self.lr, (self.mom, self.beta2) = pg[0]["lr"], pg[0]["betas"]
        self.step_count = 0
        for k, p in enumerate(self.params):
            st = sd["state"].get(k)
            o, m = self.offsets[k], p.numel()
            if st is None:
# ... 31 lines not shown
```

pdanet_amd/pointnet2_batch_cuda.py:

```python
import ctypes

import functools

import torch

from . import _lib
from . import param_cache


def _chk(t, name, dtype):
    if not isinstance(t, torch.Tensor):
        raise TypeError("%s must be a torch.Tensor" % name)
    if not t.is_cuda:
        raise RuntimeError("%s must be a CUDA(HIP) tensor -- there is no CPU path" % name)
    if not t.is_contiguous():
        raise RuntimeError("%s must be contiguous" % name)
    if t.dtype != dtype:
        raise RuntimeError("%s must be %s, got %s" % (name, dtype, t.dtype))
    return t.data_ptr()


def _numel_ok(t, n, name):
    if t.numel() < n:
        raise RuntimeError("%s has %d elements, the sizes passed need %d" % (name, t.numel(), n))


def _stream(t):
    return torch._C._cuda_getCurrentRawStream(t.device.index)


_FNS = {}


def _call(fn_name, tensor, *args):
    fn = _FNS.get(fn_name)
    if fn is None:
        fn = _FNS[fn_name] = getattr(_lib.load(), fn_name)
    idx = tensor.device.index
    if idx == torch._C._cuda_getDevice():
        st = fn(*args, torch._C._cuda_getCurrentRawStream(idx))
    else:
        with torch.cuda.device(tensor.device):
            st = fn(*args, torch._C._cuda_getCurrentRawStream(idx))
    if st != 0:
        _lib.check(st, fn_name)


F32, I32 = torch.float32, torch.int32


def ball_query_wrapper(b, n, m, radius, nsample, new_xyz, xyz, idx):
    _numel_ok(new_xyz, b * m * 3, "new_xyz"); _numel_ok(xyz, b * n * 3, "xyz")
    _numel_ok(idx, b * m * nsample, "idx")
    _call("pda_ball_query", xyz, _chk(new_xyz, "new_xyz", F32), _chk(xyz, "xyz", F32),
          _chk(idx, "idx", I32), b, n, m, float(radius), nsample)
    return 1


def ball_query_dilated_wrapper(b, n, m, max_radius, min_radius, nsample, new_xyz, xyz, idx):
    _numel_ok(new_xyz, b * m * 3, "new_xyz"); _numel_ok(xyz, b * n * 3, "xyz")
# ... 265 lines not shown
    if y is not None:
        _numel_ok(y, rows * d, "y"); yp = _chk(y, "y", F32)
    if y_bf16 is not None:
        _numel_ok(y_bf16, rows * d, "y_bf16"); yb = _chk(y_bf16, "y_bf16", BF16)
    _call("pda_layer_norm_fwd_mixed", x, _chk(x, "x", x.dtype if x.dtype == BF16 else F32), int(x.dtype == BF16), res,
          _chk(gamma, "gamma", F32), _chk(beta, "beta", F32), so, yp, yb, _chk(mean_rstd, "mean_rstd", F32), rows, d, float(eps))
    return 1


def layer_norm_bwd(x, grad_y, gamma, mean_rstd, grad_x, grad_gamma, grad_beta, scratch, rows, d, grad_y2=None, grad_x_bf16=None):
    _numel_ok(x, rows * d, "x"); _numel_ok(grad_y, rows * d, "grad_y"); _numel_ok(grad_x, rows * d, "grad_x")
    g2 = None
    if grad_y2 is not None:
        _numel_ok(grad_y2, rows * d, "grad_y2")
        g2 = _chk(grad_y2, "grad_y2", BF16 if grad_y2.dtype == BF16 else F32)
    if grad_x_bf16 is not None or (grad_y2 is not None and grad_y2.dtype == BF16):
        gxb = None
        if grad_x_bf16 is not None:
            _numel_ok(grad_x_bf16, rows * d, "grad_x_bf16"); gxb = _chk(grad_x_bf16, "grad_x_bf16", BF16)
        _call("pda_layer_norm_bwd_mixed", x, _chk(x, "x", F32), _chk(grad_y, "grad_y", F32), g2,
              int(grad_y2 is not None and grad_y2.dtype == BF16), _chk(gamma, "gamma", F32), _chk(mean_rstd, "mean_rstd", F32),
              _chk(grad_x, "grad_x", F32), gxb, _chk(grad_gamma, "grad_gamma", F32), _chk(grad_beta, "grad_beta", F32),
              _chk(scratch, "scratch", torch.uint8), rows, d)
        return 1
    _call("pda_layer_norm_bwd", x, _chk(x, "x", F32), _chk(grad_y, "grad_y", F32), g2, _chk(gamma, "gamma", F32),
          _chk(mean_rstd, "mean_rstd", F32), _chk(grad_x, "grad_x", F32), _chk(grad_gamma, "grad_gamma", F32),
          _chk(grad_beta, "grad_beta", F32), _chk(scratch, "scratch", torch.uint8), rows, d)
    return 1


_WGRAD_SCRATCH_BYTES = {}


def _wgrad_scratch_bytes(tokens, in_features, out_features):
    key = (tokens, in_features, out_features)
    nbytes = _WGRAD_SCRATCH_BYTES.get(key)
    if nbytes is None:
        if len(_WGRAD_SCRATCH_BYTES) >= 4096:
            _WGRAD_SCRATCH_BYTES.clear()
        nbytes = _WGRAD_SCRATCH_BYTES[key] = int(_lib.load().pda_linear_wgrad_scratch_bytes(tokens, in_features, out_features))
    return nbytes


@functools.lru_cache(maxsize=None)
def _split_packed_bytes(n_out, k):
    return int(_lib.load().pda_linear_split_packed_bytes(n_out, k))


@functools.lru_cache(maxsize=None)
def _cols_packed_size(n_out, k):
    return int(_lib.load().pda_linear_cols_packed_size(n_out, k))


def linear_wgrad(x, grad_out, grad_weight, grad_bias, tokens, in_features, out_features):
    _numel_ok(x, tokens * in_features, "x"); _numel_ok(grad_out, tokens * out_features, "grad_out")
    _numel_ok(grad_weight, in_features * out_features, "grad_weight")
    nbytes = _wgrad_scratch_bytes(tokens, in_features, out_features)
    scratch = torch.empty((nbytes,), dtype=torch.uint8, device=x.device)
    gb = None if grad_bias is None else _chk(grad_bias, "grad_bias", F32)
    _call("pda_linear_wgrad", x, _chk(x, "x", F32), _chk(grad_out, "grad_out", F32), _chk(grad_weight, "grad_weight", F32),
          gb, _chk(scratch, "scratch", torch.uint8), tokens, in_features, out_features)
    return 1


def linear_wgrad_bn(x, grad_out, grad_weight, tokens, in_features, out_features, x_mean_invstd, x_gamma, x_beta):
    _numel_ok(x, tokens * in_features, "x"); _numel_ok(grad_out, tokens * out_features, "grad_out")
    _numel_ok(grad_weight, in_features * out_features, "grad_weight"); _numel_ok(x_mean_invstd, 2 * in_features, "x_mean_invstd")
    _numel_ok(x_gamma, in_features, "x_gamma"); _numel_ok(x_beta, in_features, "x_beta")
    nbytes = _wgrad_scratch_bytes(tokens, in_features, out_features)
    scratch = torch.empty((nbytes,), dtype=torch.uint8, device=x.device)
    _call("pda_linear_wgrad_bn", x, _chk(x, "x", F32), _chk(grad_out, "grad_out", F32), _chk(grad_weight, "grad_weight", F32), None,
          _chk(scratch, "scratch", torch.uint8), tokens, in_features, out_features, _chk(x_mean_invstd, "x_mean_invstd", F32),
          _chk(x_gamma, "x_gamma", F32), _chk(x_beta, "x_beta", F32))
    return 1


def gemm_split_bn_tiles(tokens):
    return (int(tokens) + 255) // 256


def gemm_split_bn(x, wf, y, tokens, k, n_out, in_bn=None, stats_mode=0, partial=None):
    _numel_ok(x, tokens * k, "x"); _numel_ok(y, tokens * n_out, "y")
    _numel_ok(wf, _split_packed_bytes(int(n_out), int(k)), "wf")
    ib = (None, None, None)
    if in_bn is not None:
        _numel_ok(in_bn[0], 2 * k, "in_mean_invstd"); _numel_ok(in_bn[1], k, "in_gamma"); _numel_ok(in_bn[2], k, "in_beta")
        ib = tuple(_chk(t, "in_bn", F32) for t in in_bn)
    if stats_mode:
        _numel_ok(partial, gemm_split_bn_tiles(tokens) * 2 * n_out, "partial")
    _call("pda_gemm_split_bn", x, _chk(x, "x", F32), _chk(wf, "wf", torch.uint8), _chk(y, "y", F32), tokens, k, n_out, ib[0], ib[1], ib[2],
          int(stats_mode), None if partial is None else _chk(partial, "partial", torch.float64))
    return 1


def gemm_split_maxpool(x, wf, bias, out, tokens, k, n_out, ns, relu=True):
    _numel_ok(x, tokens * k, "x"); _numel_ok(out, (tokens // ns) * n_out, "out")
    _numel_ok(wf, _split_packed_bytes(int(n_out), int(k)), "wf")
    if bias is not None:
        _numel_ok(bias, n_out, "bias")
    _call("pda_gemm_split_maxpool", x, _chk(x, "x", F32), _chk(wf, "wf", torch.uint8), None if bias is None else _chk(bias, "bias", F32),
          _chk(out, "out", F32), tokens, k, n_out, ns, 1 if relu else 0)
    return 1


def gemm_split_gather(point_rows, xyz, new_xyz, idx, w1, bias1, wf, bias2, y, b, n, m, ns, k, n_out, relu=True):
    t = b * m * ns
    _numel_ok(point_rows, b * n * k, "point_rows"); _numel_ok(xyz, b * n * 3, "xyz"); _numel_ok(new_xyz, b * m * 3, "new_xyz")
    _numel_ok(idx, t, "idx"); _numel_ok(y, t * n_out, "y"); _numel_ok(wf, _split_packed_bytes(int(n_out), int(k)), "wf")
    if w1.dim() != 2 or w1.shape[0] != k or w1.shape[1] < 3:
        raise RuntimeError("w1 must be (k, 3 + c)")
    _call("pda_gemm_split_gather", y, _chk(point_rows, "point_rows", F32), _chk(xyz, "xyz", F32), _chk(new_xyz, "new_xyz", F32),
          _chk(idx, "idx", I32), _chk(w1, "w1", F32), int(w1.shape[1]), None if bias1 is None else _chk(bias1, "bias1", F32),
          _chk(wf, "wf", torch.uint8), None if bias2 is None else _chk(bias2, "bias2", F32), _chk(y, "y", F32), b, n, m, ns, k, n_out,
          1 if relu else 0)
    return 1


def bn_stats_fwd(x, running_mean, running_var, mean_invstd, scratch, rows, c, eps, momentum):
    _numel_ok(x, rows * c, "x"); _numel_ok(mean_invstd, 2 * c, "mean_invstd")
    rm = None if running_mean is None else _chk(running_mean, "running_mean", F32)
    rv = None if running_var is None else _chk(running_var, "running_var", F32)
    _buffers_written(rm)
    _call("pda_bn_stats_fwd", x, _chk(x, "x", F32), rm, rv, _chk(mean_invstd, "mean_invstd", F32), _chk(scratch, "scratch", torch.uint8),
          rows, c, float(eps), float(momentum))
    return 1


# ... 212 lines not shown
    _call("pda_max_pool_scatter_ragged", grad_out, _chk(grad_out, "grad_out", F32), _chk(arg, "arg", torch.uint8),
          _chk(rowmap, "rowmap", I32), _chk(off, "off", I32), _chk(grad_x, "grad_x", F32), tokens, groups, nsample, d)
    return 1


def group_attention_ragged_fwd(qkv, cnt, off, out, lse, tokens, num_groups, seq, heads, head_dim):
    _numel_ok(qkv, tokens * 3 * heads * head_dim, "qkv"); _numel_ok(out, tokens * heads * head_dim, "out")
    _numel_ok(lse, num_groups * heads * seq, "lse"); _numel_ok(cnt, num_groups, "cnt"); _numel_ok(off, num_groups + 1, "off")
    _call("pda_group_attention_ragged_fwd", qkv, _chk(qkv, "qkv", F32), _chk(cnt, "cnt", I32), _chk(off, "off", I32),
          _chk(out, "out", F32), _chk(lse, "lse", F32), tokens, num_groups, seq, heads, head_dim)
    return 1


def group_attention_ragged_bwd(qkv, grad_out, lse, cnt, off, grad_qkv, tokens, num_groups, seq, heads, head_dim):
    _numel_ok(qkv, tokens * 3 * heads * head_dim, "qkv"); _numel_ok(grad_qkv, tokens * 3 * heads * head_dim, "grad_qkv")
    _numel_ok(grad_out, tokens * heads * head_dim, "grad_out"); _numel_ok(lse, num_groups * heads * seq, "lse")
    _call("pda_group_attention_ragged_bwd", qkv, _chk(qkv, "qkv", F32), _chk(grad_out, "grad_out", F32), _chk(lse, "lse", F32),
          _chk(cnt, "cnt", I32), _chk(off, "off", I32), _chk(grad_qkv, "grad_qkv", F32), tokens, num_groups, seq, heads, head_dim)
    return 1


def linear_cols_pack(w, n_out, k, transposed_source=False, gather_order=False):
    lib = _lib.load()
    wf = torch.empty((_cols_packed_size(int(n_out), int(k)),), dtype=F32, device=w.device)
    _numel_ok(w, n_out * k, "w")
    _call("pda_linear_cols_pack", w, _chk(w, "w", F32), _chk(wf, "wf", F32), n_out, k, 1 if transposed_source else 0,
          1 if gather_order else 0)
    return wf


def linear_cols(x, wf, y, tokens, k, n_out):
    _numel_ok(x, tokens * k, "x"); _numel_ok(y, tokens * n_out, "y")
    _numel_ok(wf, _cols_packed_size(int(n_out), int(k)), "wf")
    _call("pda_linear_cols", x, _chk(x, "x", F32), _chk(wf, "wf", F32), _chk(y, "y", F32), tokens, k, n_out)
    return 1


def linear_split_pack(w, n_out, k, transposed_source=False):
    lib = _lib.load()
    wf = torch.empty((_split_packed_bytes(int(n_out), int(k)),), dtype=torch.uint8, device=w.device)
    _numel_ok(w, n_out * k, "w")
    _call("pda_linear_split_pack", w, _chk(w, "w", F32), _chk(wf, "wf", torch.uint8), n_out, k, 1 if transposed_source else 0)
    return wf


def linear_split_pack_both(w, n_out, k):
    wf = torch.empty((_split_packed_bytes(int(n_out), int(k)),), dtype=torch.uint8, device=w.device)
    wft = torch.empty((_split_packed_bytes(int(k), int(n_out)),), dtype=torch.uint8, device=w.device)
    _numel_ok(w, n_out * k, "w")
    _call("pda_linear_split_pack_both", w, _chk(w, "w", F32), _chk(wf, "wf", torch.uint8), _chk(wft, "wft", torch.uint8), n_out, k)
    return wf, wft


def linear_split(x, wf, bias, y, tokens, k, n_out, relu=False):
    _numel_ok(x, tokens * k, "x"); _numel_ok(y, tokens * n_out, "y")
    _numel_ok(wf, _split_packed_bytes(int(n_out), int(k)), "wf")
    if bias is not None:
        _numel_ok(bias, n_out, "bias")
    _call("pda_linear_split", x, _chk(x, "x", F32), _chk(wf, "wf", torch.uint8), None if bias is None else _chk(bias, "bias", F32),
          _chk(y, "y", F32), tokens, k, n_out, 1 if relu else 0)
    return 1


def gemm_split(x, wf, bias, y, tokens, k, n_out, relu=False, accumulate=False):
    _numel_ok(x, tokens * k, "x"); _numel_ok(y, tokens * n_out, "y")
    _numel_ok(wf, _split_packed_bytes(int(n_out), int(k)), "wf")
    if bias is not None:
        _numel_ok(bias, n_out, "bias")
    _call("pda_gemm_split", x, _chk(x, "x", F32), _chk(wf, "wf", torch.uint8), None if bias is None else _chk(bias, "bias", F32),
          _chk(y, "y", F32), tokens, k, n_out, 1 if relu else 0, 1 if accumulate else 0)
    return 1


def sa_gather_linear(xyz, new_xyz, feats_pm, idx, wf, y, b, n, m, c, nsample, n_out):
    _numel_ok(xyz, b * n * 3, "xyz"); _numel_ok(new_xyz, b * m * 3, "new_xyz"); _numel_ok(feats_pm, b * n * c, "feats_pm")
    _numel_ok(idx, b * m * nsample, "idx"); _numel_ok(y, b * m * nsample * n_out, "y")
    _numel_ok(wf, _cols_packed_size(int(n_out), 3 + int(c)), "wf")
    _call("pda_sa_gather_linear", xyz, _chk(xyz, "xyz", F32), _chk(new_xyz, "new_xyz", F32), _chk(feats_pm, "feats_pm", F32),
          _chk(idx, "idx", I32), _chk(wf, "wf", F32), _chk(y, "y", F32), b, n, m, c, nsample, n_out)
    return 1


@functools.lru_cache(maxsize=None)
def sa_small_train_workspace_bytes():
    return int(_lib.load().pda_sa_small_train_workspace_bytes())


@functools.lru_cache(maxsize=None)
def sa_small_train_supported(c, ns, c1, c2, c3, tokens):
    return bool(_lib.load().pda_sa_small_train_supported(int(c), int(ns), int(c1), int(c2), int(c3), int(tokens)))


def _ptr_array(ptrs):
    return (ctypes.c_void_p * len(ptrs))(*ptrs)


def sa_small_train_fwd(xyz, new_xyz, feat_pm, idx, weights, gammas, betas, running_means, running_vars, eps, momentum,
                       workspace, out, zmax, arg, b, n, m, c, ns):
    c1, c2, c3 = (int(w.shape[0]) for w in weights)
    tokens = b * m * ns
    _numel_ok(xyz, b * n * 3, "xyz"); _numel_ok(new_xyz, b * m * 3, "new_xyz"); _numel_ok(idx, tokens, "idx")
    _numel_ok(out, b * m * c3, "out"); _numel_ok(zmax, b * m * c3, "zmax"); _numel_ok(arg, b * m * c3, "arg")
    _numel_ok(workspace, sa_small_train_workspace_bytes(), "workspace")
    assert weights[0].shape[1] == 3 + c and weights[1].shape[1] == c1 and weights[2].shape[1] == c2
    if feat_pm is not None:
        _numel_ok(feat_pm, b * n * c, "feat_pm")
    rm = [None if t is None else _chk(t, "running_mean", F32) for t in running_means]
    rv = [None if t is None else _chk(t, "running_var", F32) for t in running_vars]
    _buffers_written(rm[0] or rm[1] or rm[2])
    _call("pda_sa_small_train_fwd", xyz, _chk(xyz, "xyz", F32), _chk(new_xyz, "new_xyz", F32),
          None if feat_pm is None else _chk(feat_pm, "feat_pm", F32), _chk(idx, "idx", I32),
          _chk(weights[0], "w1", F32), _chk(weights[1], "w2", F32), _chk(weights[2], "w3", F32),
          _ptr_array([_chk(t, "gamma", F32) for t in gammas]), _ptr_array([_chk(t, "beta", F32) for t in betas]),
          _ptr_array(rm), _ptr_array(rv), (ctypes.c_float * 3)(*[float(e) for e in eps]),
          (ctypes.c_float * 3)(*[float(x) for x in momentum]), _chk(workspace, "workspace", torch.uint8),
          _chk(out, "out", F32), _chk(zmax, "zmax", F32), _chk(arg, "arg", torch.uint8), b, n, m, c, ns, c1, c2, c3)
    return 1


def sa_small_train_bwd(xyz, new_xyz, feat_pm, idx, grad_out, zmax, arg, workspace, dz2, dz1, dws, dgammas, dbetas, b, n, m, c, ns):
    c1, c2, c3 = (int(w.shape[0]) for w in dws)
# ... 38 lines not shown
```

pdanet_amd/pointnet2_utils.py:

```python
from typing import List, Tuple

import os

import torch
import torch.nn as nn
from torch.autograd import Function

from . import _lib
from . import param_cache
from . import pointnet2_batch_cuda as pointnet2

_fwd = torch.amp.custom_fwd(device_type="cuda", cast_inputs=torch.float32)
_bwd = torch.amp.custom_bwd(device_type="cuda")


class FarthestPointSampling(Function):

    @staticmethod
    @_fwd
    def forward(ctx, xyz: torch.Tensor, npoint: int) -> torch.Tensor:
        assert xyz.is_contiguous()
        B, N, _ = xyz.size()
        output = torch.empty((B, npoint), dtype=torch.int32, device=xyz.device)
        temp = torch.full((B, N), 1e10, dtype=torch.float32, device=xyz.device)
        pointnet2.farthest_point_sampling_wrapper(B, N, npoint, xyz, temp, output)
        ctx.mark_non_differentiable(output)
        return output

    @staticmethod
    def backward(ctx, a=None):
        return None, None


farthest_point_sample = furthest_point_sample = FarthestPointSampling.apply


class FurthestPointSamplingWithDist(Function):

    @staticmethod
    @_fwd
    def forward(ctx, xyz: torch.Tensor, npoint: int) -> torch.Tensor:
        assert xyz.is_contiguous()
        B, N, _ = xyz.size()
        output = torch.empty((B, npoint), dtype=torch.int32, device=xyz.device)
        temp = torch.full((B, N), 1e10, dtype=torch.float32, device=xyz.device)
        pointnet2.furthest_point_sampling_with_dist_wrapper(B, N, npoint, xyz, temp, output)
        ctx.mark_non_differentiable(output)
        return output

    @staticmethod
    def backward(ctx, a=None):
        return None, None


furthest_point_sample_with_dist = FurthestPointSamplingWithDist.apply


class GatherOperation(Function):

    @staticmethod
    @_fwd
    def forward(ctx, features: torch.Tensor, idx: torch.Tensor) -> torch.Tensor:
        assert features.is_contiguous()
# ... 513 lines not shown


ROWS_IN_REGISTERS_MAX_TOKENS = int(os.environ.get("PDA_ROWS_MAX_TOKENS", "98304"))


def _rows_in_registers(tokens, k, n_out):
    return k <= 256 and n_out % 128 == 0 and n_out <= 2048 and tokens < ROWS_IN_REGISTERS_MAX_TOKENS


_PLANES = param_cache.Store(under_capture=False, weights_only=True)


def _split_planes(w, transposed=False):
    n_out, k = w.shape
    wd = w.detach()

    def pack(t):
        src = wd if wd.is_contiguous() else wd.contiguous()
        return pointnet2.linear_split_pack(src, k, n_out, transposed_source=True) if t else pointnet2.linear_split_pack(src, n_out, k)
    pair = _PLANES.get_at(w, lambda: [None, None], extra=(n_out, k)) if wd.is_contiguous() else None
    slot = 1 if transposed else 0
    if pair is not None and pair[slot] is not None:
        return pair[slot]
    if pair is None or param_cache.owning_parameter(w) is None:
        return pack(transposed)
    if w.requires_grad and n_out % 32 == 0 and k >= 128:
        pair[:] = pointnet2.linear_split_pack_both(wd, n_out, k)
    else:
        pair[slot] = pack(transposed)
    return pair[slot]


def _gemm_nt(x2d, w, bias=None, relu=False):
    n_out, k = w.shape
    if _split_gemm_ok(x2d, k) and w.dtype == torch.float32 and n_out >= 128:
        x2d = x2d.contiguous()
        T = x2d.shape[0]
        y = torch.empty((T, n_out), dtype=torch.float32, device=x2d.device)
        wf = _split_planes(w)
        bias = None if bias is None else bias.detach().contiguous()
        if _rows_in_registers(T, k, n_out):
            pointnet2.linear_split(x2d, wf, bias, y, T, k, n_out, relu=relu)
        else:
            pointnet2.gemm_split(x2d, wf, bias, y, T, k, n_out, relu=relu)
        return y
    if relu and bias is not None:
        return torch._addmm_activation(bias, x2d, w.t())
    y = torch.nn.functional.linear(x2d, w, bias)
    return torch.relu_(y) if relu else y


def _gemm_nn(g2d, w, acc=None):
    n, k_out = w.shape
    if _split_gemm_ok(g2d, n) and w.dtype == torch.float32 and k_out >= 128:
        g2d = g2d.contiguous()
        T = g2d.shape[0]
        y = acc if acc is not None else torch.empty((T, k_out), dtype=torch.float32, device=g2d.device)
        wf = _split_planes(w, transposed=True)
        if acc is None and _rows_in_registers(T, n, k_out):
            pointnet2.linear_split(g2d, wf, None, y, T, n, k_out)
        else:
            pointnet2.gemm_split(g2d, wf, None, y, T, n, k_out, accumulate=acc is not None)
        return y
    if acc is not None:
        return acc.addmm_(g2d, w)
    return g2d.mm(w)


def _mm_nt(x2d, w, bf16):
    if bf16:
        return torch.mm(_b16(x2d), _b16p(w).t(), out_dtype=torch.float32)
    return x2d.mm(w.t())


def _mm_nn(g2d, w, bf16, acc=None):
    if bf16:
        gb, wb = _b16(g2d), _b16p(w)
        if acc is not None:
            return torch.addmm(acc, gb, wb, out_dtype=torch.float32)
        return torch.mm(gb, wb, out_dtype=torch.float32)
    if acc is not None:
        return acc.addmm_(g2d, w)
    return g2d.mm(w)


def _lin(x, w, b, bf16, keep=False):
    if not bf16:
        y = torch.nn.functional.linear(x, w, b)
        return (y, x.reshape(-1, x.shape[-1])) if keep else y
    xb = _b16(x.reshape(-1, x.shape[-1]))
    y = _mm_nt(xb, w, True)
    if b is not None:
        y.add_(b)
    y = y.view(*x.shape[:-1], w.shape[0])
    return (y, xb) if keep else y


class LinearBF16(Function):

    @staticmethod
    def forward(ctx, x, weight, bias, out_bf16=False):
        xb = _b16(x.reshape(-1, x.shape[-1]))
        if out_bf16:
            wb = _b16p(weight)
            y = torch.mm(xb, wb.t()) if bias is None else torch.addmm(_b16p(bias), xb, wb.t())
        else:
            y = _mm_nt(xb, weight, True)
            if bias is not None:
                y.add_(bias)
        ctx.save_for_backward(xb, weight)
        ctx.has_bias, ctx.x_shape, ctx.x_bf16 = bias is not None, x.shape, x.dtype == torch.bfloat16
        return y.view(*x.shape[:-1], weight.shape[0])

    @staticmethod
    def backward(ctx, grad_out):
        xb, weight = ctx.saved_tensors
        n_out, n_in = weight.shape
        g2 = _b16(grad_out.reshape(-1, n_out))
        gx = gw = gb = None
        if ctx.needs_input_grad[0]:
            gx = (torch.mm(g2, _b16p(weight)) if ctx.x_bf16 else _mm_nn(g2, weight, True)).view(ctx.x_shape)
        if ctx.needs_input_grad[1] or (ctx.has_bias and ctx.needs_input_grad[2]):
            gw, gb = _wgrad(xb, g2, weight, ctx.has_bias, True)
        return gx, gw, gb, None


def linear(x, weight, bias=None, out_bf16=False):
    if weight.dim() == 2 and _dense_bf16(x, weight):
        if torch.is_grad_enabled():
            return LinearBF16.apply(x, weight, bias, out_bf16)
        return _lin(x, weight, bias, True)
    assert not out_bf16 and x.dtype == torch.float32, "bf16 boundary tensors exist only between dense-bf16 operators"
    if LINEAR_WGRAD_KERNEL and LinearLongTokens.supported(x, weight):
        return LinearLongTokens.apply(x, weight, bias)
    return torch.nn.functional.linear(x, weight, bias)


LINEAR_WGRAD_KERNEL = True


def _wgrad_bf16(xb, gb, want_bias):
    T, n_in = xb.shape
    n_out = gb.shape[1]
    tiles = max(1, (n_in // 128) * (n_out // 128))
    S = 64
    while S > 16 and S * tiles > 768:
        S //= 2
    while S > 1 and (T % S or T // S < 512):
        S //= 2
    if S > 1:
        gw = torch.bmm(gb.view(S, T // S, n_out).transpose(1, 2), xb.view(S, T // S, n_in), out_dtype=torch.float32).sum(0)
    else:
        gw = torch.mm(gb.t(), xb, out_dtype=torch.float32)
    if not want_bias:
        return gw, None
    if n_out % 8 == 0 and n_out <= 2048 and gb.is_contiguous():
        gbias = torch.empty((n_out,), dtype=torch.float32, device=gb.device)
        pointnet2.colsum_bf16(gb, gbias, T, n_out)
        return gw, gbias
    return gw, gb.sum(0, dtype=torch.float32)


def _wgrad(x2d, g2d, weight, want_bias, bf16=False):
    if bf16:
        return _wgrad_bf16(_b16(x2d), _b16(g2d), want_bias)
    if LINEAR_WGRAD_KERNEL and LinearLongTokens.kernel_wins(x2d, weight):
        gw = torch.empty_like(weight)
        gb = torch.empty((weight.shape[0],), dtype=torch.float32, device=x2d.device) if want_bias else None
        pointnet2.linear_wgrad(x2d, g2d, gw, gb, x2d.shape[0], weight.shape[1], weight.shape[0])
        return gw, gb
    return g2d.t().mm(x2d), (g2d.sum(0) if want_bias else None)


class TransformerBlock(Function):

    @staticmethod
    def supported(x, heads):
        g, s_, d = x.shape
        return (LayerNormResidual.supported(x, d) and d % heads == 0 and s_ in GroupAttention.SUPPORTED_SEQ
                and d // heads in GroupAttention.SUPPORTED_HD and not torch.is_autocast_enabled())

    @staticmethod
    def forward(ctx, x, n1w, n1b, in_w, in_b, out_w, out_b, n2w, n2b, w1, b1, w2, b2, heads, eps1, eps2, pool):
        bf16 = _dense_bf16(x)
        x = x.contiguous()
        G, S, D = x.shape
        T, hd = G * S, D // heads
        dev = x.device
        f32 = dict(dtype=torch.float32, device=dev)
        src1, ssum, src2 = torch.empty_like(x), torch.empty_like(x), torch.empty_like(x)
        st1, st2 = torch.empty((T, 2), **f32), torch.empty((T, 2), **f32)
        lse = torch.empty((G, heads, S), **f32)
        if bf16:
            b16 = dict(dtype=torch.bfloat16, device=dev)
            src1_s, src2_s = torch.empty((T, D), **b16), torch.empty((T, D), **b16)
            pointnet2.layer_norm_fwd(x, None, n1w, n1b, None, src1, st1, T, D, eps1, y_bf16=src1_s)
            qkv = torch.addmm(_b16p(in_b), src1_s, _b16p(in_w).t())
            a_s = torch.empty((T, D), **b16)
            pointnet2.group_attention_fwd(qkv, a_s, lse, G, S, heads, hd)
            proj = torch.addmm(_b16p(out_b), a_s, _b16p(out_w).t())
            pointnet2.layer_norm_fwd(proj, src1, n2w, n2b, ssum, src2, st2, T, D, eps2, y_bf16=src2_s)
            del proj
            h = h_s = torch._addmm_activation(_b16p(b1), src2_s, _b16p(w1).t())
            ffn = torch.addmm(_b16p(b2), h, _b16p(w2).t()).view(G, S, D)
        else:
            pointnet2.layer_norm_fwd(x, None, n1w, n1b, None, src1, st1, T, D, eps1)
            qkv = _gemm_nt(src1.view(T, D), in_w, in_b).view(G, S, 3 * D)
            a = torch.empty((G, S, D), **f32)
            pointnet2.group_attention_fwd(qkv, a, lse, G, S, heads, hd)
            proj = _gemm_nt(a.view(T, D), out_w, out_b).view(G, S, D)
            pointnet2.layer_norm_fwd(proj, src1, n2w, n2b, ssum, src2, st2, T, D, eps2)
            del proj
            h = _gemm_nt(src2.view(T, D), w1, b1, relu=True).view(G, S, -1)
            ffn = _gemm_nt(h.view(T, -1), w2, b2).view(G, S, D)
            src1_s, a_s, src2_s, h_s = src1.view(T, D), a.view(T, D), src2.view(T, D), h.view(T, -1)
        if pool:
            y = torch.empty((G, D), **f32)
            arg = torch.empty((G, D), dtype=torch.uint8, device=dev)
            pointnet2.add_max_pool(src2, ffn, y, arg, G, S, D)
        else:
            y = src2 + ffn
            arg = torch.empty((0,), dtype=torch.uint8, device=dev)
# ... 109 lines not shown
        x2, weight = ctx.saved_tensors
        n_out, k = weight.shape
        g2 = grad_out.contiguous().view(-1, n_out)
        T = g2.shape[0]
        gx = gw = None
        if ctx.needs_input_grad[0]:
            if n_out in (256, 512) and k % 128 == 0:
                gx = torch.empty((T, k), dtype=torch.float32, device=g2.device)
                _lin_cols(g2, weight.contiguous(), gx, T, n_out, k, True)
            else:
                gx = _gemm_nn(g2, weight)
            gx = gx.view(ctx.x_shape)
        if ctx.needs_input_grad[1]:
            gw = _wgrad(x2, g2, weight, False)[0]
        return gx, gw


class SaGatherLinear(Function):

    @staticmethod
    def supported(xyz, feats_pm, weight):
        return (SA_MFMA_TRAIN and xyz.is_cuda and feats_pm is not None and feats_pm.dtype == torch.float32 and feats_pm.shape[-1] == 256
                and weight.shape[1] == 259 and weight.shape[0] % 128 == 0 and weight.shape[0] <= 1024
                and not torch.is_autocast_enabled() and not DENSE_BF16)

    @staticmethod
    def forward(ctx, xyz, new_xyz, feats_pm, idx, weight):
        B, N, _ = xyz.shape
        M, ns = idx.shape[1], idx.shape[2]
        C, n_out = feats_pm.shape[-1], weight.shape[0]
        xyz, new_xyz, feats_pm = xyz.contiguous(), new_xyz.contiguous(), feats_pm.contiguous()
        y = torch.empty((B, M, ns, n_out), dtype=torch.float32, device=xyz.device)
        wf = pointnet2.linear_cols_pack(weight.contiguous(), n_out, 3 + C, gather_order=True)
        _sa_timed(2.0 * B * M * ns * (3 + C) * n_out,
                  lambda: pointnet2.sa_gather_linear(xyz, new_xyz, feats_pm, idx, wf, y, B, N, M, C, ns, n_out))
        ctx.save_for_backward(xyz, new_xyz, feats_pm, idx, weight)
        return y

    @staticmethod
    def backward(ctx, grad_out):
        xyz, new_xyz, feats_pm, idx, weight = ctx.saved_tensors
        B, M, ns = idx.shape
        n_out, C, N = weight.shape[0], feats_pm.shape[-1], xyz.shape[1]
        g2 = grad_out.contiguous().view(-1, n_out)
        T = g2.shape[0]
        g_new = g_feats = gw = None
        with torch.no_grad():
            if ctx.needs_input_grad[4] or ctx.needs_input_grad[1]:
                gw = torch.empty_like(weight)
                g_new = torch.empty_like(new_xyz) if ctx.needs_input_grad[1] else None
                pointnet2.sa_xyz_grad(g2, xyz, new_xyz, idx, weight.contiguous(), gw, g_new, B, N, M, ns, n_out)
            if ctx.needs_input_grad[4]:
                gf_in = group_rows(feats_pm, idx).view(T, C)
                gw[:, 3:] = _wgrad(gf_in, g2, torch.empty((n_out, C), dtype=weight.dtype, device=weight.device), False)[0]
                del gf_in
            else:
                gw = None
            if ctx.needs_input_grad[2]:
                gxf = _gemm_nn(g2, weight[:, 3:].contiguous())
                g_feats = torch.zeros_like(feats_pm)
                pointnet2.group_rows_grad(B, feats_pm.shape[1], C, M * ns, gxf, idx, g_feats)
        return None, g_new, g_feats, None, gw


SA_POINT_LINEAR = os.environ.get("PDA_SA_POINT_LINEAR", "1") != "0"


class SaPointLinear(Function):

    @staticmethod
    def supported(xyz, feats_pm, weight):
        return (SA_POINT_LINEAR and SPLIT_GEMM and SaGatherLinear.supported(xyz, feats_pm, weight) and weight.shape[0] in (128, 256, 512, 1024)
                and feats_pm.shape[0] * feats_pm.shape[1] >= SPLIT_GEMM_MIN_TOKENS)

    @staticmethod
    def forward(ctx, xyz, new_xyz, feats_pm, idx, weight):
        B, N, _ = xyz.shape
        M, ns = idx.shape[1], idx.shape[2]
        C, n_out = feats_pm.shape[-1], weight.shape[0]
        xyz, new_xyz, feats_pm, idx = xyz.contiguous(), new_xyz.contiguous(), feats_pm.contiguous(), idx.contiguous()
        w = weight.detach().contiguous()
        w_f = w[:, 3:].contiguous()
        rows = _gemm_nt(feats_pm.view(B * N, C), w_f)
        z = torch.empty((B, M, ns, n_out), dtype=torch.float32, device=xyz.device)
        pointnet2.sa_point_gather(rows, xyz, new_xyz, idx, w, z, B, N, M, ns, n_out)
        ctx.save_for_backward(xyz, new_xyz, feats_pm, idx, weight)
        return z

    @staticmethod
    def backward(ctx, grad_out):
        xyz, new_xyz, feats_pm, idx, weight = ctx.saved_tensors
        B, M, ns = idx.shape
        n_out, C, N = weight.shape[0], feats_pm.shape[-1], xyz.shape[1]
        g2 = grad_out.contiguous().view(-1, n_out)
        g_new = g_feats = gw = None
        with torch.no_grad():
            w = weight.contiguous()
            if ctx.needs_input_grad[4] or ctx.needs_input_grad[1]:
                gw = torch.empty_like(weight)
                g_new = torch.empty_like(new_xyz) if ctx.needs_input_grad[1] else None
                pointnet2.sa_xyz_grad(g2, xyz, new_xyz, idx, w, gw, g_new, B, N, M, ns, n_out)
            if ctx.needs_input_grad[4] or ctx.needs_input_grad[2]:
                g_pts = torch.zeros((B, N, n_out), dtype=torch.float32, device=g2.device)
                pointnet2.group_rows_grad(B, N, n_out, M * ns, g2, idx, g_pts)
                g_pts = g_pts.view(B * N, n_out)
                if ctx.needs_input_grad[4]:
                    gw[:, 3:] = _wgrad(feats_pm.view(B * N, C), g_pts, torch.empty((n_out, C), dtype=weight.dtype, device=weight.device), False)[0]
                if ctx.needs_input_grad[2]:
                    g_feats = _gemm_nn(g_pts, w[:, 3:].contiguous()).view(B, N, C)
            if not ctx.needs_input_grad[4]:
                gw = None
        return None, g_new, g_feats, None, gw


SA_WIDE_INFER_SPLIT = os.environ.get("PDA_SA_WIDE_INFER_SPLIT", "1") != "0"
SA_WIDE_INFER_GATHER_IN_GEMM = os.environ.get("PDA_SA_WIDE_INFER_GATHER_IN_GEMM", "1") != "0"


def sa_wide_scale_infer(xyz, new_xyz, feats_pm, idx, folded):
    (w1, b1), (w2, b2), (w3, b3) = folded
    B, N, _ = xyz.shape
    M, ns = idx.shape[1], idx.shape[2]
    C = feats_pm.shape[-1]
    T = B * M * ns
    c1, c2, c3 = w1.shape[0], w2.shape[0], w3.shape[0]
    if not (SA_WIDE_INFER_SPLIT and SPLIT_GEMM and not DENSE_BF16 and w1.shape[1] == 3 + C and C % 32 == 0 and c1 in (128, 256, 512, 1024)
            and c1 % 32 == 0 and c2 % 128 == 0 and c3 % 128 == 0 and B * N >= SPLIT_GEMM_MIN_TOKENS and T >= SPLIT_GEMM_MIN_TOKENS):
        return None
    out = []

    def run():
        rows = _gemm_nt(feats_pm.reshape(B * N, C), w1[:, 3:].contiguous())
        if SA_WIDE_INFER_GATHER_IN_GEMM and c1 % 32 == 0 and c1 <= 1024:
            y2 = torch.empty((T, c2), dtype=torch.float32, device=xyz.device)
            pointnet2.gemm_split_gather(rows, xyz.contiguous(), new_xyz.contiguous(), idx.contiguous(), w1.contiguous(), b1.detach().contiguous(),
                                        _split_planes(w2), b2.detach().contiguous(), y2, B, N, M, ns, c1, c2, relu=True)
        else:
            y1 = torch.empty((T, c1), dtype=torch.float32, device=xyz.device)
            pointnet2.sa_point_gather(rows, xyz.contiguous(), new_xyz.contiguous(), idx.contiguous(), w1, y1, B, N, M, ns, c1, bias=b1, relu=True)
            y2 = _gemm_nt(y1, w2, b2, relu=True)
            del y1
        if ns in (16, 32, 64) and c2 % 32 == 0:
            pooled = torch.empty((B, M, c3), dtype=torch.float32, device=xyz.device)
            pointnet2.gemm_split_maxpool(y2, _split_planes(w3), b3.detach().contiguous(), pooled, T, c2, c3, ns, relu=True)
            out.append(pooled)
            return
        y3 = _gemm_nt(y2, w3, b3, relu=True)
        del y2
        out.append(y3.view(B, M, ns, c3).amax(dim=2))
    _sa_timed(2.0 * T * (c1 * c2 + c2 * c3), run, "bf16x6_infer")
    return out[0]


SA_SMALL_TRAIN = True
FUSED_WIDE_CHAIN_OK = True


class SaSmallChainTrain(Function):

    @staticmethod
# ... 120 lines not shown
            _sa_timed(2.0 * T * k * n_out, lambda: pointnet2.gemm_split_bn(z_in, wf, z, T, k, n_out, in_bn=(mi_in, gi, bi), stats_mode=1,
                                                                           partial=part), "bf16x6")
            mi = torch.empty((2 * n_out,), dtype=torch.float32, device=dev)
            pointnet2.bn_finalize_fwd(part, tiles, n_out, T, bn.eps, bn.momentum, mi, st[0], st[1])
            return z, mi
        z2, mi2 = layer(z1, mi1, c1, w2, c2, bns[1], stats[1], gs[0], bs[0])
        z3, mi3 = layer(z2, mi2, c2, w3, c3, bns[2], stats[2], gs[1], bs[1])
        out = torch.empty((B, M, c3), dtype=torch.float32, device=dev)
        arg = torch.empty((B, M, c3), dtype=torch.uint8, device=dev)
        pointnet2.bn_relu_max_pool_apply(z3, gs[2], bs[2], mi3, out, arg, B * M, ns, c3)
        ctx.save_for_backward(xyz, new_xyz, feats_pm, idx, w1, w2, w3, g1, b1, g2, b2, g3, b3, z1, z2, z3, mi1, mi2, mi3, arg)
        return out

    @staticmethod
    def backward(ctx, grad_out):
        xyz, new_xyz, feats_pm, idx, w1, w2, w3, g1, b1, g2, b2, g3, b3, z1, z2, z3, mi1, mi2, mi3, arg = ctx.saved_tensors
        B, M, ns = idx.shape
        N, C = xyz.shape[1], feats_pm.shape[-1]
        c1, c2, c3 = w1.shape[0], w2.shape[0], w3.shape[0]
        T = B * M * ns
        dev = xyz.device
        tiles = pointnet2.gemm_split_bn_tiles(T)
        with torch.no_grad():
            g1c, b1c, g2c, b2c, g3c, b3c = (t.contiguous() for t in (g1, b1, g2, b2, g3, b3))
            gz3 = torch.empty((T, c3), dtype=torch.float32, device=dev)
            dg3, db3 = torch.empty_like(g3c), torch.empty_like(b3c)
            scratch = torch.empty((pointnet2.bn_relu_scratch_bytes(c3),), dtype=torch.uint8, device=dev)
            pointnet2.bn_relu_max_pool_bwd(z3, grad_out.contiguous().float(), arg, g3c, b3c, mi3, gz3, dg3, db3, scratch, B * M, ns, c3)

            def layer(gz, w, z_in, mi_in, gi, bi, k_in, n_out):
                dw = torch.empty((n_out, k_in), dtype=torch.float32, device=dev)
                ga = torch.empty((T, k_in), dtype=torch.float32, device=dev)
                if WIDE_CHAIN_DGRAD_FIRST:
                    _lin_cols(gz, w, ga, T, n_out, k_in, True)
                    pointnet2.linear_wgrad_bn(z_in, gz, dw, T, k_in, n_out, mi_in, gi, bi)
                else:
                    pointnet2.linear_wgrad_bn(z_in, gz, dw, T, k_in, n_out, mi_in, gi, bi)
                    _lin_cols(gz, w, ga, T, n_out, k_in, True)
                dg, db = torch.empty_like(gi), torch.empty_like(bi)
                scratch = torch.empty((pointnet2.bn_relu_scratch_bytes(k_in),), dtype=torch.uint8, device=dev)
                pointnet2.bn_relu_bwd(z_in, ga, gi, bi, mi_in, ga, dg, db, scratch, T, k_in)
                return dw, ga, dg, db
            dw3, gz2, dg2, db2 = layer(gz3, w3, z2, mi2, g2c, b2c, c2, c3)
            del gz3
            dw2, gz1, dg1, db1 = layer(gz2, w2, z1, mi1, g1c, b1c, c1, c2)
            del gz2
            w1c = w1.contiguous()
            dw1 = torch.empty_like(w1c)
            g_new = torch.empty_like(new_xyz) if ctx.needs_input_grad[1] else None
            pointnet2.sa_xyz_grad(gz1, xyz, new_xyz, idx, w1c, dw1, g_new, B, N, M, ns, c1)
            g_pts = torch.zeros((B, N, c1), dtype=torch.float32, device=dev)
            pointnet2.group_rows_grad(B, N, c1, M * ns, gz1, idx, g_pts)
            g_pts = g_pts.view(B * N, c1)
            dw1[:, 3:] = _wgrad(feats_pm.view(B * N, C), g_pts, torch.empty((c1, C), dtype=torch.float32, device=dev), False)[0]
            g_feats = _gemm_nn(g_pts, w1c[:, 3:].contiguous()).view(B, N, C) if ctx.needs_input_grad[2] else None
        return None, g_new, g_feats, None, dw1, dw2, dw3, dg1, db1, dg2, db2, dg3, db3, None


def sa_wide_chain_train(xyz, new_xyz, feats_pm, idx, mlp):
    layers = list(mlp)
    convs, bns = [layers[0], layers[3], layers[6]], [layers[1], layers[4], layers[7]]
    for bn in bns:
        bump_bn_counter(bn)
    return SaWideChainTrain.apply(xyz, new_xyz, feats_pm, idx, convs[0].weight.flatten(1), convs[1].weight.flatten(1),
                                  convs[2].weight.flatten(1), bns[0].weight, bns[0].bias, bns[1].weight, bns[1].bias,
                                  bns[2].weight, bns[2].bias, bns)


RAGGED_TOKENS = True
RAGGED_MAX_FRACTION = 0.85


class RaggedPlan:
    __slots__ = ("cnt", "off", "rowmap", "roww", "tokens", "groups", "nsample")

    def __init__(self, cnt, off, rowmap, roww, tokens, groups, nsample):
        self.cnt, self.off, self.rowmap, self.roww = cnt, off, rowmap, roww
        self.tokens, self.groups, self.nsample = tokens, groups, nsample

    @property
    def fraction(self):
        return self.tokens / float(self.groups * self.nsample)


def ragged_plan_parts(idxs):
    parts = []
    for idx in idxs:
        G, ns = idx.shape[0] * idx.shape[1], idx.shape[2]
        cnt = torch.empty((G,), dtype=torch.int32, device=idx.device)
        off = torch.empty((G + 1,), dtype=torch.int32, device=idx.device)
        rowmap = torch.empty((G * ns,), dtype=torch.int32, device=idx.device)
        roww = torch.empty((G * ns,), dtype=torch.float32, device=idx.device)
        pointnet2.ragged_plan(idx, cnt, off, rowmap, G, ns, roww)
        parts.append((cnt, off, rowmap, roww, G, ns))
    return parts, torch.stack([p[1][-1] for p in parts])


def ragged_plans_from(parts, totals):
    return [RaggedPlan(c, o, r[:u], w[:u], int(u), G, ns) for (c, o, r, w, G, ns), u in zip(parts, totals)]


def ragged_plans(idxs):
    parts, totals = ragged_plan_parts(idxs)
    return ragged_plans_from(parts, totals.tolist())


ASSEMBLE_BWD_TOKEN_PARALLEL = os.environ.get("PDA_ASSEMBLE_BWD_TOKEN_PARALLEL", "1") != "0"
# ... 406 lines not shown
```

Measured before the change: 120.6 scenes/s.

## Overlap weight-gradient GEMMs on a low-priority side stream during backward

```diff
diff --git a/include/pda_pointnet2.h b/include/pda_pointnet2.h
--- a/include/pda_pointnet2.h
+++ b/include/pda_pointnet2.h
@@ -101,6 +101,10 @@
                      int relu, pda_stream_t stream);
 int pda_gemm_split(const float *x, const void *wf, const float *bias, float *y, int64_t tokens, int k, int n_out,
                    int relu, int accumulate, pda_stream_t stream);
+int pda_linear_split_res(const float *x, const void *wf, const float *bias, const float *residual, float *y, int64_t tokens,
+                         int k, int n_out, int relu, pda_stream_t stream);
+int pda_gemm_split_res(const float *x, const void *wf, const float *bias, const float *residual, float *y, int64_t tokens,
+                       int k, int n_out, int relu, int tile, pda_stream_t stream);
 int pda_sa_mlp_packed_size(int rows, int cols, int first_layer);
 int pda_sa_mlp_pack_weights(const float *w, float *wf, int rows, int cols, int first_layer,
                             pda_stream_t stream);
diff --git a/include/pda_train.h b/include/pda_train.h
--- a/include/pda_train.h
+++ b/include/pda_train.h
@@ -54,6 +54,13 @@
 int pda_linear_wgrad_bn(const float *x, const float *grad_out, float *grad_weight, float *grad_bias, void *scratch,
                         int64_t tokens, int in_features, int out_features, const float *x_mean_invstd,
                         const float *x_gamma, const float *x_beta, pda_stream_t stream);
+int pda_linear_wgrad_bounded(const float *x, const float *grad_out, float *grad_weight, float *grad_bias, void *scratch,
+                             int64_t tokens, int in_features, int out_features, const float *x_mean_invstd,
+                             const float *x_gamma, const float *x_beta, int max_workgroups, pda_stream_t stream);
+
+int pda_side_queue_fork(pda_stream_t main_stream, pda_stream_t *side_stream);
+int pda_side_queue_join(pda_stream_t main_stream);
+int pda_side_queue_pending(void);
 
 int64_t pda_gemm_split_bn_tiles(int64_t tokens);
 int pda_gemm_split_bn(const float *x, const void *wf, float *y, int64_t tokens, int k, int n_out,
diff --git a/pdanet_amd/_lib.py b/pdanet_amd/_lib.py
--- a/pdanet_amd/_lib.py
+++ b/pdanet_amd/_lib.py
@@ -74,6 +74,8 @@
     "pda_linear_split_pack_both": [_vp, _vp, _vp, _i, _i, _vp],
     "pda_linear_split": [_vp, _vp, _vp, _vp, ctypes.c_int64, _i, _i, _i, _vp],
     "pda_gemm_split": [_vp, _vp, _vp, _vp, ctypes.c_int64, _i, _i, _i, _i, _vp],
+    "pda_linear_split_res": [_vp, _vp, _vp, _vp, _vp, ctypes.c_int64, _i, _i, _i, _vp],
+    "pda_gemm_split_res": [_vp, _vp, _vp, _vp, _vp, ctypes.c_int64, _i, _i, _i, _i, _vp],
     "pda_sa_mlp_packed_size": [_i, _i, _i],
     "pda_sa_mlp_pack_weights": [_vp, _vp, _i, _i, _i, _vp],
     "pda_grad_norm": [_vp, ctypes.c_int64, _vp, _vp, _vp],
@@ -93,6 +95,10 @@
     "pda_linear_wgrad_form": [ctypes.c_int64, _i, _i],
     "pda_linear_wgrad": [_vp, _vp, _vp, _vp, _vp, ctypes.c_int64, _i, _i, _vp],
     "pda_linear_wgrad_bn": [_vp, _vp, _vp, _vp, _vp, ctypes.c_int64, _i, _i, _vp, _vp, _vp, _vp],
+    "pda_linear_wgrad_bounded": [_vp, _vp, _vp, _vp, _vp, ctypes.c_int64, _i, _i, _vp, _vp, _vp, _i, _vp],
+    "pda_side_queue_fork": [_vp, ctypes.POINTER(_vp)],
+    "pda_side_queue_join": [_vp],
+    "pda_side_queue_pending": [],
     "pda_gemm_split_bn_tiles": [ctypes.c_int64],
     "pda_gemm_split_bn": [_vp, _vp, _vp, ctypes.c_int64, _i, _i, _vp, _vp, _vp, _i, _vp, _vp],
     "pda_gemm_split_maxpool": [_vp, _vp, _vp, _vp, ctypes.c_int64, _i, _i, _i, _i, _vp],
diff --git a/pdanet_amd/csrc/gemm_split.hip b/pdanet_amd/csrc/gemm_split.hip
--- a/pdanet_amd/csrc/gemm_split.hip
+++ b/pdanet_amd/csrc/gemm_split.hip
@@ -46,6 +46,7 @@
     const uint4* wf;
     const float* bias;
     float* y;
+    const float* res;
     int64_t tokens;
     int k, n_out, chunks, relu;
     int cpb;
@@ -57,7 +58,7 @@
 #define GS_MARK(i) do {} while (0)
 #endif
 
-template <int KS>
+template <int KS, bool RES>
 __global__ __launch_bounds__(256) __attribute__((amdgpu_waves_per_eu(1, 1)))
 void lin_split_kernel(const LinSplitParams p) {
     constexpr int G = KS % 4 == 0 ? 4 : 2;
@@ -106,8 +107,11 @@
     auto store_one = [&](const gs_f32x16 (&res)[4], int chunk, int n) {
         const int r = n >> 4, i = n & 15, t = (i & 3) + 8 * (i >> 2);
         float v = res[r][i] + bias_s[chunk * 128 + r * 32 + j];
+        float* row = p.y + (tok0 + t) * p.n_out + chunk * 128 + r * 32;
+        if constexpr (RES) {
+            if (whole || t < left) v += (p.res + (tok0 + t) * p.n_out + chunk * 128 + r * 32)[lane_off];
+        }
         if (p.relu) v = fmaxf(v, 0.f);
-        float* row = p.y + (tok0 + t) * p.n_out + chunk * 128 + r * 32;
         if (whole) row[lane_off] = v;
         else if (t < left) row[lane_off] = v;
     };
@@ -191,7 +195,8 @@
     const float* bias;
     float* y;
     int64_t tokens;
-    int k, n_out, chunks, ksteps, relu, accum;
+    int k, n_out, chunks, ksteps, relu;
+    const float* res;
     const float* in_mi;
     const float* in_g;
     const float* in_b;
@@ -310,7 +315,7 @@
                 if (tok < p.tokens) {
                     float* dst = p.y + tok * p.n_out + col;
                     float v = acc[tt][ot][i] + bias;
-                    if (p.accum) v += *dst;
+                    if (p.res) v += p.res[tok * p.n_out + col];
                     if (p.relu) v = fmaxf(v, 0.f);
 #ifdef GS_NOSTORE
                     if (v == 12345.678f)
@@ -552,7 +557,7 @@
                 if (tok < p.tokens) {
                     float* dst = p.y + tok * p.n_out + col;
                     float v = acc[tt][ot][i] + bias;
-                    if (p.accum) v += *dst;
+                    if (p.res) v += p.res[tok * p.n_out + col];
                     if (p.relu) v = fmaxf(v, 0.f);
 #ifdef GS_NOSTORE
                     if (v == 12345.678f)
@@ -618,6 +623,11 @@
 
 PDA_API int pda_linear_split(const float* x, const void* wf, const float* bias, float* y, int64_t tokens, int k, int n_out,
                              int relu, pda_stream_t stream) {
+    return pda_linear_split_res(x, wf, bias, nullptr, y, tokens, k, n_out, relu, stream);
+}
+
+PDA_API int pda_linear_split_res(const float* x, const void* wf, const float* bias, const float* residual, float* y, int64_t tokens,
+                                 int k, int n_out, int relu, pda_stream_t stream) {
     PDA_REQUIRE(tokens >= 0 && k > 0 && n_out > 0, "pda_linear_split: bad size");
     if (tokens == 0) return PDA_OK;
     PDA_REQUIRE(x && wf && y && (((uintptr_t)x | (uintptr_t)wf | (uintptr_t)y | (uintptr_t)bias) & 15) == 0,
@@ -628,7 +638,7 @@
     }
     pda::LinSplitParams p{};
     p.x = x; p.wf = (const uint4*)wf; p.bias = bias; p.y = y; p.tokens = tokens; p.k = k; p.n_out = n_out; p.chunks = n_out / 128;
-    p.relu = relu;
+    p.relu = relu; p.res = residual;
 #ifdef GS_PROFILE
     p.dbg = (unsigned long long*)bias; p.bias = nullptr;
 #endif
@@ -638,7 +648,8 @@
     const dim3 grid((unsigned)tiles, (unsigned)pda::divup(p.chunks, p.cpb)), block(256);
     const hipStream_t s = (hipStream_t)stream;
     switch (k / 16) {
-#define PDA_GS_CASE(KS) case KS: hipLaunchKernelGGL((pda::lin_split_kernel<KS>), grid, block, 0, s, p); break
+#define PDA_GS_CASE(KS) case KS: if (residual) hipLaunchKernelGGL((pda::lin_split_kernel<KS, true>), grid, block, 0, s, p); \
+                                 else hipLaunchKernelGGL((pda::lin_split_kernel<KS, false>), grid, block, 0, s, p); break
         PDA_GS_CASE(2); PDA_GS_CASE(4); PDA_GS_CASE(6); PDA_GS_CASE(8); PDA_GS_CASE(12); PDA_GS_CASE(16); PDA_GS_CASE(24); PDA_GS_CASE(32);
 #undef PDA_GS_CASE
         default:
@@ -650,6 +661,12 @@
 
 PDA_API int pda_gemm_split(const float* x, const void* wf, const float* bias, float* y, int64_t tokens, int k, int n_out,
                            int relu, int accumulate, pda_stream_t stream) {
+    return pda_gemm_split_res(x, wf, bias, accumulate ? y : nullptr, y, tokens, k, n_out, relu, 0, stream);
+}
+
+PDA_API int pda_gemm_split_res(const float* x, const void* wf, const float* bias, const float* residual, float* y, int64_t tokens,
+                               int k, int n_out, int relu, int tile, pda_stream_t stream) {
+    PDA_REQUIRE(tile == 0 || tile == 128 || tile == 256, "pda_gemm_split: tile=%d", tile);
     PDA_REQUIRE(tokens >= 0 && k > 0 && n_out > 0, "pda_gemm_split: bad size");
     if (tokens == 0) return PDA_OK;
     PDA_REQUIRE(x && wf && y && (((uintptr_t)x | (uintptr_t)wf) & 15) == 0, "pda_gemm_split: null or misaligned pointer");
@@ -659,7 +676,7 @@
     }
     pda::GemmSplitParams p{};
     p.x = x; p.wf = (const uint4*)wf; p.bias = bias; p.y = y; p.tokens = tokens; p.k = k; p.n_out = n_out;
-    p.chunks = pda::divup(n_out, 128); p.ksteps = pda::divup(k, 32) * 2; p.relu = relu; p.accum = accumulate;
+    p.chunks = pda::divup(n_out, 128); p.ksteps = pda::divup(k, 32) * 2; p.relu = relu; p.res = residual;
     const int64_t blocks = pda::divup64(tokens, 128) * p.chunks;
     PDA_REQUIRE(blocks < (1ll << 31), "pda_gemm_split: too many tiles");
     const int packed_steps = p.ksteps;
@@ -668,7 +685,8 @@
         pda::set_error("pda_gemm_split: K=%d must be a multiple of 32 (packed planes come in pairs of K steps)", k);
         return PDA_ERR_UNSUPPORTED;
     }
-    static const int force = getenv("PDA_GEMM_SPLIT_TILE") ? atoi(getenv("PDA_GEMM_SPLIT_TILE")) : 0;
+    static const int env_force = getenv("PDA_GEMM_SPLIT_TILE") ? atoi(getenv("PDA_GEMM_SPLIT_TILE")) : 0;
+    const int force = tile ? tile : env_force;
     const int64_t wide_blocks = pda::divup64(tokens, 256) * ((p.chunks + 1) / 2);
     if (force == 256 || (force != 128 && wide_blocks >= 200 && (p.chunks % 2 == 0 || p.chunks >= 5))) {
         static pda::PerDevice<bool> lds_ok;
diff --git a/pdanet_amd/csrc/side_queue.hip b/pdanet_amd/csrc/side_queue.hip
--- /dev/null
+++ b/pdanet_amd/csrc/side_queue.hip
@@ -0,0 +1,100 @@
+#include "pda_common.h"
+
+#include <mutex>
+
+namespace pda {
+
+constexpr int SQ_EVENTS = 8;
+
+struct SideQueue {
+    std::mutex mu;
+    hipStream_t stream = nullptr;
+    hipEvent_t events[SQ_EVENTS] = {};
+    int next_event = 0;
+    int pending = 0;
+    bool ready = false;
+};
+
+static SideQueue g_side_queues[PerDevice<int>::MAX_DEV];
+
+static bool side_queue_init(SideQueue& q) {
+    if (q.ready) return true;
+    int least = 0, greatest = 0;
+    if (hipDeviceGetStreamPriorityRange(&least, &greatest) != hipSuccess) return false;
+    if (hipStreamCreateWithPriority(&q.stream, hipStreamNonBlocking, least) != hipSuccess) return false;
+    for (int i = 0; i < SQ_EVENTS; ++i)
+        if (hipEventCreateWithFlags(&q.events[i], hipEventDisableTiming) != hipSuccess) return false;
+    q.ready = true;
+    return true;
+}
+
+static SideQueue* side_queue_here() {
+    int dev = 0;
+    if (hipGetDevice(&dev) != hipSuccess || dev < 0 || dev >= PerDevice<int>::MAX_DEV) return nullptr;
+    return &g_side_queues[dev];
+}
+
+}
+
+PDA_API int pda_side_queue_fork(pda_stream_t main_stream, pda_stream_t* side_stream) {
+    PDA_REQUIRE(side_stream, "pda_side_queue_fork: null pointer");
+    hipStream_t main = (hipStream_t)main_stream;
+    hipStreamCaptureStatus cap = hipStreamCaptureStatusNone;
+    if (hipStreamIsCapturing(main, &cap) != hipSuccess) {
+        (void)hipGetLastError();
+        pda::set_error("pda_side_queue_fork: hipStreamIsCapturing failed");
+        return PDA_ERR_LAUNCH;
+    }
+    if (cap != hipStreamCaptureStatusNone) {
+        *side_stream = main_stream;
+        return PDA_OK;
+    }
+    pda::SideQueue* q = pda::side_queue_here();
+    PDA_REQUIRE(q, "pda_side_queue_fork: no current device");
+    std::lock_guard<std::mutex> lock(q->mu);
+    if (!pda::side_queue_init(*q)) {
+        (void)hipGetLastError();
+        pda::set_error("pda_side_queue_fork: could not create the low-priority stream");
+        return PDA_ERR_LAUNCH;
+    }
+    hipEvent_t ev = q->events[q->next_event];
+    q->next_event = (q->next_event + 1) % pda::SQ_EVENTS;
+    if (hipEventRecord(ev, main) != hipSuccess || hipStreamWaitEvent(q->stream, ev, 0) != hipSuccess) {
+        (void)hipGetLastError();
+        pda::set_error("pda_side_queue_fork: event record / wait failed");
+        return PDA_ERR_LAUNCH;
+    }
+    ++q->pending;
+    *side_stream = (pda_stream_t)q->stream;
+    return PDA_OK;
+}
+
+PDA_API int pda_side_queue_join(pda_stream_t main_stream) {
+    pda::SideQueue* q = pda::side_queue_here();
+    PDA_REQUIRE(q, "pda_side_queue_join: no current device");
+    std::lock_guard<std::mutex> lock(q->mu);
+    if (!q->ready || q->pending == 0) return PDA_OK;
+    hipStreamCaptureStatus cap = hipStreamCaptureStatusNone;
+    if (hipStreamIsCapturing((hipStream_t)main_stream, &cap) != hipSuccess) {
+        (void)hipGetLastError();
+        pda::set_error("pda_side_queue_join: hipStreamIsCapturing failed");
+        return PDA_ERR_LAUNCH;
+    }
+    if (cap != hipStreamCaptureStatusNone) return PDA_OK;
+    hipEvent_t ev = q->events[q->next_event];
+    q->next_event = (q->next_event + 1) % pda::SQ_EVENTS;
+    if (hipEventRecord(ev, q->stream) != hipSuccess || hipStreamWaitEvent((hipStream_t)main_stream, ev, 0) != hipSuccess) {
+        (void)hipGetLastError();
+        pda::set_error("pda_side_queue_join: event record / wait failed");
+        return PDA_ERR_LAUNCH;
+    }
+    q->pending = 0;
+    return PDA_OK;
+}
+
+PDA_API int pda_side_queue_pending(void) {
+    pda::SideQueue* q = pda::side_queue_here();
+    if (!q) return 0;
+    std::lock_guard<std::mutex> lock(q->mu);
+    return q->pending;
+}
diff --git a/pdanet_amd/csrc/wgrad.hip b/pdanet_amd/csrc/wgrad.hip
--- a/pdanet_amd/csrc/wgrad.hip
+++ b/pdanet_amd/csrc/wgrad.hip
@@ -17,13 +17,16 @@
                  : "=&s"(keep) : "v"(gsrc), "s"(dst) : "memory");
 }
 
+template <bool LOOP>
 __global__ __launch_bounds__(256) void wgrad_kernel(const float* __restrict__ X, const float* __restrict__ G,
                                                     float* __restrict__ part_w, float* __restrict__ part_b, int64_t T, int M,
                                                     int N, int tiles_m, int tiles_n, int S, int64_t KS, int nblocks) {
     __shared__ __attribute__((aligned(16))) float ldsG[2][WG_KC][WG_TILE];
     __shared__ __attribute__((aligned(16))) float ldsX[2][WG_KC][WG_TILE];
     const int per_xcd = (nblocks + 7) / 8;
-    const int logical = (int)(blockIdx.x & 7) * per_xcd + (int)(blockIdx.x >> 3);
+    int in_xcd = (int)(blockIdx.x >> 3);
+  do {
+    const int logical = (int)(blockIdx.x & 7) * per_xcd + in_xcd;
     if (logical >= nblocks) return;
     const int tiles = tiles_m * tiles_n;
     const int tile = logical % tiles, s = logical / tiles;
@@ -152,6 +155,7 @@
             if (h == 0 && n < N) part_b[(size_t)s * N + n] = v;
         }
     }
+  } while (LOOP && (in_xcd += (int)(gridDim.x >> 3)) < per_xcd);
 }
 
 #ifndef WSP_ABL
@@ -159,14 +163,16 @@
 #endif
 constexpr int WSP_TILE_U4 = 2 * 8 * 3 * 64;
 
-template <bool XBN>
+template <bool XBN, bool LOOP>
 __global__ __launch_bounds__(512, 1)
 void wgrad_split_kernel(const float* __restrict__ X, const float* __restrict__ G, float* __restrict__ part_w,
                         float* __restrict__ part_b, int64_t T, int M, int N, int tiles_m, int tiles_n, int S, int64_t KS,
                         int nblocks, const float* __restrict__ x_mi, const float* __restrict__ x_g, const float* __restrict__ x_b) {
     extern __shared__ uint4 wsp_planes[];
     const int per_xcd = (nblocks + 7) / 8;
-    const int logical = (int)(blockIdx.x & 7) * per_xcd + (int)(blockIdx.x >> 3);
+    int in_xcd = (int)(blockIdx.x >> 3);
+  do {
+    const int logical = (int)(blockIdx.x & 7) * per_xcd + in_xcd;
     if (logical >= nblocks) return;
     const int tiles = tiles_m * tiles_n;
     const int tile = logical % tiles, s = logical / tiles;
@@ -330,6 +336,8 @@
         const float v = bsum + __shfl_xor(bsum, 32);
         if (h == 0) part_b[(size_t)s * N + n0 + 32 * w + c] = v;
     }
+    if (LOOP) __syncthreads();
+  } while (LOOP && (in_xcd += (int)(gridDim.x >> 3)) < per_xcd);
 }
 
 __device__ __forceinline__ float sum_slices(const float* __restrict__ part, int S, int64_t stride, int64_t e, bool live, int slice,
@@ -503,7 +511,16 @@
 
 namespace pda {
 static int linear_wgrad(const float* x, const float* grad_out, float* grad_weight, float* grad_bias, void* scratch, int64_t tokens,
-                        int in_features, int out_features, pda_stream_t stream, const float* x_mi, const float* x_g, const float* x_b);
+                        int in_features, int out_features, pda_stream_t stream, const float* x_mi, const float* x_g, const float* x_b,
+                        int max_workgroups = 0);
+
+static int wgrad_grid(int nblocks, int max_workgroups, bool& loop) {
+    const int per_xcd = divup(nblocks, 8);
+    int g8 = per_xcd;
+    if (max_workgroups > 0 && max_workgroups / 8 < g8) g8 = max_workgroups / 8 > 0 ? max_workgroups / 8 : 1;
+    loop = g8 < per_xcd;
+    return g8 * 8;
+}
 }
 
 PDA_API int pda_linear_wgrad(const float* x, const float* grad_out, float* grad_weight, float* grad_bias, void* scratch,
@@ -522,8 +539,24 @@
     return pda::linear_wgrad(x, grad_out, grad_weight, grad_bias, scratch, tokens, in_features, out_features, stream, x_mean_invstd, x_gamma, x_beta);
 }
 
+PDA_API int pda_linear_wgrad_bounded(const float* x, const float* grad_out, float* grad_weight, float* grad_bias, void* scratch,
+                                     int64_t tokens, int in_features, int out_features, const float* x_mean_invstd, const float* x_gamma,
+                                     const float* x_beta, int max_workgroups, pda_stream_t stream) {
+    PDA_REQUIRE(max_workgroups >= 0, "pda_linear_wgrad_bounded: max_workgroups=%d", max_workgroups);
+    if (x_mean_invstd) {
+        PDA_REQUIRE(x_gamma && x_beta, "pda_linear_wgrad_bounded: null pointer");
+        if (pda_linear_wgrad_form(tokens, in_features, out_features) != 2) {
+            pda::set_error("pda_linear_wgrad_bounded: tokens=%lld in=%d out=%d does not run on the split form", (long long)tokens, in_features, out_features);
+            return PDA_ERR_UNSUPPORTED;
+        }
+    }
+    return pda::linear_wgrad(x, grad_out, grad_weight, grad_bias, scratch, tokens, in_features, out_features, stream,
+                             x_mean_invstd, x_mean_invstd ? x_gamma : nullptr, x_mean_invstd ? x_beta : nullptr, max_workgroups);
+}
+
 int pda::linear_wgrad(const float* x, const float* grad_out, float* grad_weight, float* grad_bias, void* scratch, int64_t tokens,
-                             int in_features, int out_features, pda_stream_t stream, const float* x_mi, const float* x_g, const float* x_b) {
+                             int in_features, int out_features, pda_stream_t stream, const float* x_mi, const float* x_g, const float* x_b,
+                             int max_workgroups) {
     const int M = in_features, N = out_features;
     PDA_REQUIRE(tokens >= 1 && M >= 4 && N >= 4 && (M & 3) == 0 && (N & 3) == 0,
                 "pda_linear_wgrad: tokens=%lld in=%d out=%d (features must be multiples of 4)", (long long)tokens, M, N);
@@ -553,17 +586,23 @@
         const int nblocks = S * tm * tn;
         float* part_w = (float*)scratch;
         float* part_b = part_w + (size_t)S * N * M;
+        constexpr int lds_bytes = 2 * pda::WSP_TILE_U4 * 16;
         static pda::PerDevice<bool> lds_ok;
         const bool ok = lds_ok.get([] {
-            return hipFuncSetAttribute((const void*)pda::wgrad_split_kernel<false>, hipFuncAttributeMaxDynamicSharedMemorySize, 2 * pda::WSP_TILE_U4 * 16) == hipSuccess &&
-                   hipFuncSetAttribute((const void*)pda::wgrad_split_kernel<true>, hipFuncAttributeMaxDynamicSharedMemorySize, 2 * pda::WSP_TILE_U4 * 16) == hipSuccess; });
-        PDA_REQUIRE(ok, "pda_linear_wgrad: %d bytes of dynamic LDS refused", 2 * pda::WSP_TILE_U4 * 16);
-        if (x_mi)
-            hipLaunchKernelGGL(pda::wgrad_split_kernel<true>, dim3(pda::divup(nblocks, 8) * 8), dim3(512), 2 * pda::WSP_TILE_U4 * 16, st,
-                               x, grad_out, part_w, grad_bias ? part_b : (float*)nullptr, tokens, M, N, tm, tn, S, KS, nblocks, x_mi, x_g, x_b);
-        else
-            hipLaunchKernelGGL(pda::wgrad_split_kernel<false>, dim3(pda::divup(nblocks, 8) * 8), dim3(512), 2 * pda::WSP_TILE_U4 * 16, st,
-                               x, grad_out, part_w, grad_bias ? part_b : (float*)nullptr, tokens, M, N, tm, tn, S, KS, nblocks, x_mi, x_g, x_b);
+            const void* fns[4] = {(const void*)pda::wgrad_split_kernel<false, false>, (const void*)pda::wgrad_split_kernel<true, false>,
+                                  (const void*)pda::wgrad_split_kernel<false, true>, (const void*)pda::wgrad_split_kernel<true, true>};
+            for (const void* f : fns)
+                if (hipFuncSetAttribute(f, hipFuncAttributeMaxDynamicSharedMemorySize, lds_bytes) != hipSuccess) return false;
+            return true; });
+        PDA_REQUIRE(ok, "pda_linear_wgrad: %d bytes of dynamic LDS refused", lds_bytes);
+        bool loop;
+        const int grid = pda::wgrad_grid(nblocks, max_workgroups, loop);
+        float* pb = grad_bias ? part_b : (float*)nullptr;
+#define PDA_WSP_LAUNCH(XBN, LOOP) hipLaunchKernelGGL((pda::wgrad_split_kernel<XBN, LOOP>), dim3(grid), dim3(512), lds_bytes, st, \
+                                                     x, grad_out, part_w, pb, tokens, M, N, tm, tn, S, KS, nblocks, x_mi, x_g, x_b)
+        if (x_mi) { if (loop) PDA_WSP_LAUNCH(true, true); else PDA_WSP_LAUNCH(true, false); }
+        else { if (loop) PDA_WSP_LAUNCH(false, true); else PDA_WSP_LAUNCH(false, false); }
+#undef PDA_WSP_LAUNCH
         const int64_t nm = (int64_t)N * M;
         hipLaunchKernelGGL(pda::wgrad_reduce_kernel, dim3((unsigned)pda::divup64(nm, 64)), dim3(1024), 0, st, part_w, part_b,
                            grad_weight, grad_bias, S, nm, N);
@@ -573,8 +612,14 @@
     const int nblocks = S * tm * tn;
     float* part_w = (float*)scratch;
     float* part_b = part_w + (size_t)S * N * M;
-    hipLaunchKernelGGL(pda::wgrad_kernel, dim3(pda::divup(nblocks, 8) * 8), dim3(256), 0, st, x, grad_out, part_w,
-                       grad_bias ? part_b : (float*)nullptr, tokens, M, N, tm, tn, S, KS, nblocks);
+    bool loop;
+    const int grid = pda::wgrad_grid(nblocks, max_workgroups, loop);
+    if (loop)
+        hipLaunchKernelGGL(pda::wgrad_kernel<true>, dim3(grid), dim3(256), 0, st, x, grad_out, part_w,
+                           grad_bias ? part_b : (float*)nullptr, tokens, M, N, tm, tn, S, KS, nblocks);
+    else
+        hipLaunchKernelGGL(pda::wgrad_kernel<false>, dim3(grid), dim3(256), 0, st, x, grad_out, part_w,
+                           grad_bias ? part_b : (float*)nullptr, tokens, M, N, tm, tn, S, KS, nblocks);
     const int64_t nm = (int64_t)N * M;
     hipLaunchKernelGGL(pda::wgrad_reduce_kernel, dim3((unsigned)pda::divup64(nm, 64)), dim3(1024), 0, st, part_w, part_b, grad_weight,
                        grad_bias, S, nm, N);
diff --git a/pdanet_amd/optimization.py b/pdanet_amd/optimization.py
--- a/pdanet_amd/optimization.py
+++ b/pdanet_amd/optimization.py
@@ -6,6 +6,7 @@
 
 from . import _lib
 from . import param_cache
+from . import wgrad_queue
 
 BN_TYPES = (nn.BatchNorm1d, nn.BatchNorm2d, nn.BatchNorm3d, nn.SyncBatchNorm)
 
@@ -129,6 +130,7 @@
 
     def exchange_gradients(self):
         import torch.distributed as dist
+        wgrad_queue.join()
         if self._gather:
             self._gather_grads()
         if self._dp_world == 1:
@@ -140,6 +142,10 @@
             self.flat_g.mul_(1.0 / self._dp_world)
 
     def zero_grad(self, set_to_none=False):
+        if not set_to_none:
+            wgrad_queue.enable(False)
+        elif wgrad_queue.ARMED_BY_OPTIMIZER:
+            wgrad_queue.enable(True, once=True)
         if set_to_none:
             for p in self._all:
                 p.grad = None
@@ -152,6 +158,7 @@
             self.flat_g.zero_()
 
     def _gather_grads(self):
+        wgrad_queue.join()
         self.flat_g.zero_()
         dsts, srcs = [], []
         for p, v in zip(self._all, self._grad_views):
@@ -167,6 +174,7 @@
         if self.flat_p.device.type != "cuda":
             raise _lib.PdaError("FlatAdamOneCycle.step needs the parameters on the GPU (no CPU path)")
         lib = _lib.load()
+        wgrad_queue.join()
         if self._gather:
             self._gather_grads()
         if self._dp_world > 1:
diff --git a/pdanet_amd/pointnet2_batch_cuda.py b/pdanet_amd/pointnet2_batch_cuda.py
--- a/pdanet_amd/pointnet2_batch_cuda.py
+++ b/pdanet_amd/pointnet2_batch_cuda.py
@@ -6,6 +6,7 @@
 
 from . import _lib
 from . import param_cache
+from . import wgrad_queue
 
 
 def _chk(t, name, dtype):
@@ -377,27 +378,51 @@
     return int(_lib.load().pda_linear_cols_packed_size(n_out, k))
 
 
-def linear_wgrad(x, grad_out, grad_weight, grad_bias, tokens, in_features, out_features):
-    _numel_ok(x, tokens * in_features, "x"); _numel_ok(grad_out, tokens * out_features, "grad_out")
-    _numel_ok(grad_weight, in_features * out_features, "grad_weight")
+def _wgrad_call(x, grad_out, grad_weight, grad_bias, tokens, in_features, out_features, bn, queue, max_workgroups):
     nbytes = _wgrad_scratch_bytes(tokens, in_features, out_features)
     scratch = torch.empty((nbytes,), dtype=torch.uint8, device=x.device)
     gb = None if grad_bias is None else _chk(grad_bias, "grad_bias", F32)
-    _call("pda_linear_wgrad", x, _chk(x, "x", F32), _chk(grad_out, "grad_out", F32), _chk(grad_weight, "grad_weight", F32),
-          gb, _chk(scratch, "scratch", torch.uint8), tokens, in_features, out_features)
-    return 1
-
-
-def linear_wgrad_bn(x, grad_out, grad_weight, tokens, in_features, out_features, x_mean_invstd, x_gamma, x_beta):
+    args = (_chk(x, "x", F32), _chk(grad_out, "grad_out", F32), _chk(grad_weight, "grad_weight", F32), gb,
+            _chk(scratch, "scratch", torch.uint8), tokens, in_features, out_features)
+    bn_ptrs = (None, None, None) if bn is None else tuple(_chk(t, "x_bn", F32) for t in bn)
+    side = None
+    if queue and wgrad_queue.enabled() and not wgrad_queue.inline.active():
+        side = wgrad_queue.fork(x, (x, grad_out, scratch, bn, grad_weight.untyped_storage(),
+                                    None if grad_bias is None else grad_bias.untyped_storage()))
+    if side is not None:
+        bound = wgrad_queue.MAX_WORKGROUPS if max_workgroups is None else int(max_workgroups)
+        fn = _FNS.get("pda_linear_wgrad_bounded")
+        if fn is None:
+            fn = _FNS["pda_linear_wgrad_bounded"] = _lib.load().pda_linear_wgrad_bounded
+        if x.device.index == torch._C._cuda_getDevice():
+            st = fn(*args, *bn_ptrs, bound, side)
+        else:
+            with torch.cuda.device(x.device):
+                st = fn(*args, *bn_ptrs, bound, side)
+        if st != 0:
+            _lib.check(st, "pda_linear_wgrad_bounded")
+    elif max_workgroups is not None:
+        _call("pda_linear_wgrad_bounded", x, *args, *bn_ptrs, int(max_workgroups))
+    elif bn is None:
+        _call("pda_linear_wgrad", x, *args)
+    else:
+        _call("pda_linear_wgrad_bn", x, *args, *bn_ptrs)
+    return 1
+
+
+def linear_wgrad(x, grad_out, grad_weight, grad_bias, tokens, in_features, out_features, queue=True, max_workgroups=None):
+    _numel_ok(x, tokens * in_features, "x"); _numel_ok(grad_out, tokens * out_features, "grad_out")
+    _numel_ok(grad_weight, in_features * out_features, "grad_weight")
+    return _wgrad_call(x, grad_out, grad_weight, grad_bias, tokens, in_features, out_features, None, queue, max_workgroups)
+
+
+def linear_wgrad_bn(x, grad_out, grad_weight, tokens, in_features, out_features, x_mean_invstd, x_gamma, x_beta, queue=True,
+                    max_workgroups=None):
     _numel_ok(x, tokens * in_features, "x"); _numel_ok(grad_out, tokens * out_features, "grad_out")
     _numel_ok(grad_weight, in_features * out_features, "grad_weight"); _numel_ok(x_mean_invstd, 2 * in_features, "x_mean_invstd")
     _numel_ok(x_gamma, in_features, "x_gamma"); _numel_ok(x_beta, in_features, "x_beta")
-    nbytes = _wgrad_scratch_bytes(tokens, in_features, out_features)
-    scratch = torch.empty((nbytes,), dtype=torch.uint8, device=x.device)
-    _call("pda_linear_wgrad_bn", x, _chk(x, "x", F32), _chk(grad_out, "grad_out", F32), _chk(grad_weight, "grad_weight", F32), None,
-          _chk(scratch, "scratch", torch.uint8), tokens, in_features, out_features, _chk(x_mean_invstd, "x_mean_invstd", F32),
-          _chk(x_gamma, "x_gamma", F32), _chk(x_beta, "x_beta", F32))
-    return 1
+    return _wgrad_call(x, grad_out, grad_weight, None, tokens, in_features, out_features, (x_mean_invstd, x_gamma, x_beta), queue,
+                       max_workgroups)
 
 
 def gemm_split_bn_tiles(tokens):
@@ -716,21 +741,33 @@
     return wf, wft
 
 
-def linear_split(x, wf, bias, y, tokens, k, n_out, relu=False):
+def linear_split(x, wf, bias, y, tokens, k, n_out, relu=False, residual=None):
     _numel_ok(x, tokens * k, "x"); _numel_ok(y, tokens * n_out, "y")
     _numel_ok(wf, _split_packed_bytes(int(n_out), int(k)), "wf")
     if bias is not None:
         _numel_ok(bias, n_out, "bias")
+    if residual is not None:
+        _numel_ok(residual, tokens * n_out, "residual")
+        _call("pda_linear_split_res", x, _chk(x, "x", F32), _chk(wf, "wf", torch.uint8), None if bias is None else _chk(bias, "bias", F32),
+              _chk(residual, "residual", F32), _chk(y, "y", F32), tokens, k, n_out, 1 if relu else 0)
+        return 1
     _call("pda_linear_split", x, _chk(x, "x", F32), _chk(wf, "wf", torch.uint8), None if bias is None else _chk(bias, "bias", F32),
           _chk(y, "y", F32), tokens, k, n_out, 1 if relu else 0)
     return 1
 
 
-def gemm_split(x, wf, bias, y, tokens, k, n_out, relu=False, accumulate=False):
+def gemm_split(x, wf, bias, y, tokens, k, n_out, relu=False, accumulate=False, residual=None, tile=0):
     _numel_ok(x, tokens * k, "x"); _numel_ok(y, tokens * n_out, "y")
     _numel_ok(wf, _split_packed_bytes(int(n_out), int(k)), "wf")
     if bias is not None:
         _numel_ok(bias, n_out, "bias")
+    if residual is not None or tile:
+        if residual is not None:
+            _numel_ok(residual, tokens * n_out, "residual")
+        res = _chk(residual, "residual", F32) if residual is not None else (_chk(y, "y", F32) if accumulate else None)
+        _call("pda_gemm_split_res", x, _chk(x, "x", F32), _chk(wf, "wf", torch.uint8), None if bias is None else _chk(bias, "bias", F32),
+              res, _chk(y, "y", F32), tokens, k, n_out, 1 if relu else 0, int(tile))
+        return 1
     _call("pda_gemm_split", x, _chk(x, "x", F32), _chk(wf, "wf", torch.uint8), None if bias is None else _chk(bias, "bias", F32),
           _chk(y, "y", F32), tokens, k, n_out, 1 if relu else 0, 1 if accumulate else 0)
     return 1
diff --git a/pdanet_amd/pointnet2_utils.py b/pdanet_amd/pointnet2_utils.py
--- a/pdanet_amd/pointnet2_utils.py
+++ b/pdanet_amd/pointnet2_utils.py
@@ -9,6 +9,7 @@
 from . import _lib
 from . import param_cache
 from . import pointnet2_batch_cuda as pointnet2
+from . import wgrad_queue
 
 _fwd = torch.amp.custom_fwd(device_type="cuda", cast_inputs=torch.float32)
 _bwd = torch.amp.custom_bwd(device_type="cuda")
@@ -628,18 +629,21 @@
 
 def _gemm_nn(g2d, w, acc=None):
     n, k_out = w.shape
+    fresh = acc is not None and wgrad_queue.enabled()
     if _split_gemm_ok(g2d, n) and w.dtype == torch.float32 and k_out >= 128:
         g2d = g2d.contiguous()
         T = g2d.shape[0]
-        y = acc if acc is not None else torch.empty((T, k_out), dtype=torch.float32, device=g2d.device)
+        y = acc if acc is not None and not fresh else torch.empty((T, k_out), dtype=torch.float32, device=g2d.device)
         wf = _split_planes(w, transposed=True)
         if acc is None and _rows_in_registers(T, n, k_out):
             pointnet2.linear_split(g2d, wf, None, y, T, n, k_out)
+        elif fresh:
+            pointnet2.gemm_split(g2d, wf, None, y, T, n, k_out, residual=acc.contiguous())
         else:
             pointnet2.gemm_split(g2d, wf, None, y, T, n, k_out, accumulate=acc is not None)
         return y
     if acc is not None:
-        return acc.addmm_(g2d, w)
+        return torch.addmm(acc, g2d, w) if fresh else acc.addmm_(g2d, w)
     return g2d.mm(w)
 
 
@@ -737,13 +741,17 @@
     return gw, gb.sum(0, dtype=torch.float32)
 
 
-def _wgrad(x2d, g2d, weight, want_bias, bf16=False):
+def _wgrad(x2d, g2d, weight, want_bias, bf16=False, queue=True):
     if bf16:
         return _wgrad_bf16(_b16(x2d), _b16(g2d), want_bias)
     if LINEAR_WGRAD_KERNEL and LinearLongTokens.kernel_wins(x2d, weight):
         gw = torch.empty_like(weight)
         gb = torch.empty((weight.shape[0],), dtype=torch.float32, device=x2d.device) if want_bias else None
-        pointnet2.linear_wgrad(x2d, g2d, gw, gb, x2d.shape[0], weight.shape[1], weight.shape[0])
+        if queue:
+            pointnet2.linear_wgrad(x2d, g2d, gw, gb, x2d.shape[0], weight.shape[1], weight.shape[0])
+        else:
+            with wgrad_queue.inline():
+                pointnet2.linear_wgrad(x2d, g2d, gw, gb, x2d.shape[0], weight.shape[1], weight.shape[0])
         return gw, gb
     return g2d.t().mm(x2d), (g2d.sum(0) if want_bias else None)
 
@@ -959,7 +967,7 @@
                 pointnet2.sa_xyz_grad(g2, xyz, new_xyz, idx, weight.contiguous(), gw, g_new, B, N, M, ns, n_out)
             if ctx.needs_input_grad[4]:
                 gf_in = group_rows(feats_pm, idx).view(T, C)
-                gw[:, 3:] = _wgrad(gf_in, g2, torch.empty((n_out, C), dtype=weight.dtype, device=weight.device), False)[0]
+                gw[:, 3:] = _wgrad(gf_in, g2, torch.empty((n_out, C), dtype=weight.dtype, device=weight.device), False, queue=False)[0]
                 del gf_in
             else:
                 gw = None
@@ -1012,7 +1020,8 @@
                 pointnet2.group_rows_grad(B, N, n_out, M * ns, g2, idx, g_pts)
                 g_pts = g_pts.view(B * N, n_out)
                 if ctx.needs_input_grad[4]:
-                    gw[:, 3:] = _wgrad(feats_pm.view(B * N, C), g_pts, torch.empty((n_out, C), dtype=weight.dtype, device=weight.device), False)[0]
+                    gw[:, 3:] = _wgrad(feats_pm.view(B * N, C), g_pts, torch.empty((n_out, C), dtype=weight.dtype, device=weight.device), False,
+                                        queue=False)[0]
                 if ctx.needs_input_grad[2]:
                     g_feats = _gemm_nn(g_pts, w[:, 3:].contiguous()).view(B, N, C)
             if not ctx.needs_input_grad[4]:
@@ -1239,7 +1248,7 @@
             g_pts = torch.zeros((B, N, c1), dtype=torch.float32, device=dev)
             pointnet2.group_rows_grad(B, N, c1, M * ns, gz1, idx, g_pts)
             g_pts = g_pts.view(B * N, c1)
-            dw1[:, 3:] = _wgrad(feats_pm.view(B * N, C), g_pts, torch.empty((c1, C), dtype=torch.float32, device=dev), False)[0]
+            dw1[:, 3:] = _wgrad(feats_pm.view(B * N, C), g_pts, torch.empty((c1, C), dtype=torch.float32, device=dev), False, queue=False)[0]
             g_feats = _gemm_nn(g_pts, w1c[:, 3:].contiguous()).view(B, N, C) if ctx.needs_input_grad[2] else None
         return None, g_new, g_feats, None, dw1, dw2, dw3, dg1, db1, dg2, db2, dg3, db3, None
 
diff --git a/pdanet_amd/wgrad_queue.py b/pdanet_amd/wgrad_queue.py
--- /dev/null
+++ b/pdanet_amd/wgrad_queue.py
@@ -0,0 +1,103 @@
+import ctypes
+import os
+import threading
+
+import torch
+
+from . import _lib
+
+FORCED_OFF = os.environ.get("PDA_WGRAD_QUEUE") == "0"
+ARMED_BY_OPTIMIZER = os.environ.get("PDA_WGRAD_QUEUE") == "1"
+MAX_WORKGROUPS = int(os.environ.get("PDA_WGRAD_QUEUE_WORKGROUPS", "128"))
+
+_OFF, _ON, _ONCE = 0, 1, 2
+_mode = _OFF
+_lock = threading.RLock()
+_held = []
+_main = None
+_callback_queued = False
+
+
+def enable(flag=True, once=False):
+    global _mode, _callback_queued
+    with _lock:
+        _mode = _OFF if (not flag or FORCED_OFF) else (_ONCE if once else _ON)
+        _callback_queued = False
+    if not flag:
+        join()
+
+
+def enabled():
+    return _mode != _OFF
+
+
+class inline:
+    _local = threading.local()
+
+    def __enter__(self):
+        inline._local.depth = getattr(inline._local, "depth", 0) + 1
+
+    def __exit__(self, *exc):
+        inline._local.depth -= 1
+        return False
+
+    @staticmethod
+    def active():
+        return getattr(inline._local, "depth", 0) > 0
+
+
+def pending():
+    return int(_lib.load().pda_side_queue_pending())
+
+
+def _on_device(idx, fn, *args):
+    if idx == torch._C._cuda_getDevice():
+        return fn(*args)
+    with torch.cuda.device(idx):
+        return fn(*args)
+
+
+def fork(tensor, keep):
+    global _main, _callback_queued
+    if _mode == _OFF:
+        return None
+    idx = tensor.device.index
+    main = torch._C._cuda_getCurrentRawStream(idx)
+    lib = _lib.load()
+    with _lock:
+        if not _callback_queued:
+            try:
+                torch.autograd.Variable._execution_engine.queue_callback(_end_of_backward)
+                _callback_queued = True
+            except RuntimeError:
+                if _mode == _ONCE:
+                    return None
+        if _main is not None and _main != (idx, main):
+            join()
+        side = ctypes.c_void_p()
+        _lib.check(_on_device(idx, lib.pda_side_queue_fork, main, ctypes.byref(side)), "pda_side_queue_fork")
+        if (side.value or 0) == main:
+            return None
+        _main = (idx, main)
+        _held.append(keep)
+    return side.value
+
+
+def join():
+    global _main, _callback_queued
+    with _lock:
+        _callback_queued = False
+        if _main is None:
+            return
+        idx, main = _main
+        _lib.check(_on_device(idx, _lib.load().pda_side_queue_join, main), "pda_side_queue_join")
+        _main = None
+        _held.clear()
+
+
+def _end_of_backward():
+    global _mode
+    join()
+    with _lock:
+        if _mode == _ONCE:
+            _mode = _OFF
```

Result: slower. 107.8 scenes/s (-10.6%).
